# Mahdi-Si/VAE-TEB

Hardware: AMD Instinct MI355X
Metric: train samples/sec + ELBO, 4096-pt windows, batch 256, 1/2/4/8 MI355X (higher is better)
Workload: dtype bf16 MFMA (decoder heads + conv blocks + ResidualMLP linears, LSTM recurrences f16 fwd / bf16 bwd), fp32 accumulation; fp32 LayerNorm / BatchNorm / LSTM state / front-end / optimizer

## Files before the change

include/vaeteb.h:

```cpp
#ifndef VAETEB_H
#define VAETEB_H

#include <stdint.h>

#ifdef __cplusplus
extern "C" {
#endif

#define VT_OK 0
#define VT_ERR_ARG (-1)
#define VT_ERR_LAYOUT (-2)
#define VT_ERR_HIP (-3)

#define VT_FFT_MAX_LDS 8192

const char* vt_last_error(void);
int vt_stream_fork(void* from, void* to);
int vt_stream_mark(void* stream, int* slot);
int vt_stream_wait_mark(void* stream, int slot);
int vt_abi_version(void);
int vt_arrive_reset(void* stream);
int vt_capture_info(void* stream, char* buf, int len);
int vt_set_h16_format(int fp16);
int vt_get_h16_format(void);


int vt_fe_spectrum(const float* x, int64_t rows, int N, int n_pad, int pad_left, int pad_mode, const void* tw,
                   void* xhat, void* stream);
int vt_fe_spectrum_rolled(const float* x, int64_t B, int64_t x_row_stride, int N, int n_pad, int pad_left,
                          int pad_mode, const int* shifts, int K, const void* tw, void* xhat, void* stream);

int vt_fe_lowpass(const float* x, int64_t rows, int64_t x_row_stride, int N, int n_pad, int pad_left,
                  const float* h0, int radius, int step, int start, int S, float* out, int64_t out_row_stride,
                  void* stream);

int vt_fe_wavelet(const void* xhat, int64_t B, int C, int n_pad, const float* psi, int n_items, const int* items,
                  const void* tw, int N, int pad_left, void* analytic, int n_slots, const float* h0, int radius,
                  int step, int start, int S, float* s1, int s1_channels, void* stream);

int vt_fe_pairs(const void* analytic, int64_t B, int n_slots, int N, int n_pad, int pad_left, int n_pairs,
                const int* slot_i, const int* slot_j, const float* power, const void* tw, const float* phi0, int dec,
                int start, int S, int pad_mode, float* out, void* stream);
int vt_fe_pairs_split(const void* analytic_i, int n_slots_i, const void* analytic_j, int n_slots_j, int64_t B, int K,
                      int N, int n_pad, int pad_left, int n_pairs, const int* slot_i, const int* slot_j,
                      const float* power, const void* tw, const float* phi0, int dec, int start, int S,
                      int pad_mode, float* out, void* stream);

int vt_fe_set_pairs_persist(int grid);
int vt_fe_set_pairs_direct(int on);
int vt_fe_set_pairs_half(int on);
int vt_fe_set_analytic_polar(int on);

int vt_fe_set_pairs_stamps(void* buf);

int vt_fe_normalize(const float* in, int64_t B, int C, int in_C, int S, const int* kind, const float* mean, const float* stdv,
                    float log_eps, float* out, int out_C, int out_off, void* stream);
int vt_fe_normalize_window(const float* in, int64_t B, int C, int in_C, int in_S, int s0, int S_len,
                           const int* kind, const float* mean, const float* stdv, float log_eps, float* out,
                           int out_C, int out_off, void* stream);
int vt_copy_cols(const float* src, int64_t rows, int ld_src, int src_col0, int ncols, float* dst, int ld_dst,
                 int dst_col0, void* stream);
int vt_clamp_bwd(const float* g, const float* x, int64_t n, float lo, float hi, float* gx, void* stream);
int vt_zero_ranges(float* base, int n, const int64_t* starts, const int64_t* ends, void* stream);
int vt_normalize_raw(const float* x, int64_t rows, int64_t row_stride, int N, float mean, float stdv, float* out,
                     void* stream);

#define VT_STATS_CHUNK_ROWS 32
#define VT_STATS_CHUNK_COLS 1024
int vt_stats_chunking(int* rows, int* cols);
int vt_stats_workspace_bytes(int64_t B, int C, int S_len, int64_t* bytes);
int vt_stats_accum(const float* in, int64_t B, int C, int in_C, int in_S, int s0, int S_len, const int* kind,
                   double log_eps, int64_t* count, double* sum, double* sum_sq, void* work, int64_t work_bytes,
                   void* stream);
int vt_stats_accum_raw(const float* x, int64_t rows, int64_t row_stride, int N, int64_t* count, double* sum,
                       double* sum_sq, void* work, int64_t work_bytes, void* stream);

int vt_window_flat_stats(const float* base, const int64_t* row_off, int64_t rows, int N, double tolerance,
                         int min_length, int32_t* out, void* stream);
int vt_window_gather(const float* base, const int64_t* row_off, int64_t rows, int N, float* out, void* stream);

int vt_fft(const void* in, void* out, int64_t rows, int n, int inverse, const void* tw, int tw_stride,
           void* stream);
int vt_fft_large(const void* in, void* out, void* ws, int64_t rows, int n, int inverse, const void* tw,
                 void* stream);
int vt_cdgmm(const void* A, const void* B, int b_is_real, void* C, int64_t rows, int n, void* stream);
int vt_scat_filter_sub(const void* A, int B, int64_t a_rows, int n, const int* a_idx, const float* pool,
                       const int64_t* f_off, int P, int k, void* out, void* stream);
int vt_scat_mod_spec(const void* A, int B, int64_t a_rows, int n, const int* a_idx, const float* pool,
                     const int64_t* f_off, int P, int k, const void* tw, void* out, void* stream);
int vt_scat_lowpass(const void* U, int B, int P, int n, const float* phi, int k, int i0, int i1, const int* ch,
                    int out_C, const void* tw, float* out, void* stream);
int vt_modulus_cplx(const void* in, void* out, int64_t count, void* stream);
int vt_modulus(const void* in, float* out, int64_t count, void* stream);
int vt_modulus_bwd(const void* in, const float* mod, const float* grad, void* grad_in, int64_t count, void* stream);
int vt_subsample_fourier(const void* in, void* out, int64_t rows, int n, int k, void* stream);
int vt_pad_reflect(const float* in, float* out, int64_t rows, int N, int pad_left, int pad_right, void* stream);
int vt_scat_lowpass_bwd(const float* g, int B, int P, int n, const float* phi, int k, int i0, int i1, const int* ch,
                        int out_C, const void* tw, void* gU, void* stream);
int vt_scat_mod_spec_bwd(const void* A, int B, int64_t a_rows, int n, const int* a_idx, const float* pool,
                         const int64_t* f_off, int P, int k, const void* tw, const void* gUh, void* gX,
                         void* stream);
int vt_scat_fold_bwd(const void* gX, int B, int a_rows, int n, const int* csr_ptr, const int* csr_p,
                     const float* pool, const int64_t* f_off, int P, int k, void* gA, void* stream);
int vt_modulus_cplx_bwd(const void* z, const void* G, void* out, int64_t count, void* stream);
int vt_pad_reflect_bwd(const float* g, int g_stride, float scale, float* gx, int64_t rows, int N, int pad_left,
                       int pad_right, void* stream);
int vt_subsample_fourier_bwd(const void* g, void* gx, int64_t rows, int n, int k, void* stream);


int vt_elbo_workspace_floats(void);

int vt_elbo_latent_fwd(const float* mu_c, const float* lv_q, const float* mu_y, const float* lv_p, const float* eps,
                       int64_t rows, int D, float* z, float* mu_post, float* kl, float* ws, void* stream);
int vt_elbo_latent_bwd(const float* mu_c, const float* lv_q, const float* mu_y, const float* lv_p, const float* eps,
                       int64_t rows, int D, const float* g_z, const float* g_mu_post, const float* g_kl,
                       float* g_mu_c, float* g_lv_q, float* g_mu_y, float* g_lv_p, void* stream);
int vt_elbo_output_fwd(const float* mu, const float* lv, const float* y, int64_t n_nll, const float* lin,
                       const float* t_st, const float* t_ph, int64_t rows, int c_st, int c_ph, float* g_mu,
                       float* g_lv, float* g_lin, float* nll, float* mse, float* ws, void* stream);
int vt_scale_by_device_scalar(float* x, int64_t n, const float* s, void* stream);
int vt_te_kl_rows(const float* mu_c, const float* lv_q, const float* mu_y, const float* lv_p, int64_t B, int K,
                  int64_t row_elems, float* te, float* kl, void* stream);
int vt_eval_scale_rows(const float* x, int64_t B, int K, int64_t row_elems, const float* gains, float* out,
                       void* stream);
int vt_te_latent_rows(const float* mu_c, const float* lv_q, const float* mu_y, const float* lv_p, const float* eps,
                      int64_t B, int K, int64_t row_elems, float* z, float* mu_post, float* te, float* kl,
                      void* stream);
int vt_recon_metrics_rows(const float* y, const float* pr, int64_t B, int K, int64_t n, float* out, void* stream);

int vt_grad_norm_workspace_floats(void);
int vt_grad_norm_clip(const float* g, int64_t n, float pre_scale, float max_norm, float* out2, float* ws,
                      void* stream);
int vt_grad_norm_clip_scaled(const float* g, int64_t n, float pre_scale, float max_norm, float* out3, float* ws,
                             float* scaler, float growth_factor, float backoff_factor, int growth_interval,
                             void* stream);
int vt_adamw_step(float* p, const float* g, float* m, float* v, int64_t n, float lr, float beta1, float beta2,
                  float eps, float weight_decay, int step, const float* gscale, void* stream);
int vt_adamw_step_dev(float* p, const float* g, float* m, float* v, int64_t n, float lr, float beta1, float beta2,
                      float eps, float weight_decay, int* step, float* coef, const float* gscale, void* stream);
int vt_adamw_step_dev_shadow(float* p, const float* g, float* m, float* v, int64_t n, float lr, float beta1,
                             float beta2, float eps, float weight_decay, int* step, float* coef, const float* gscale,
                             int n_tiled, const int64_t* tiled_off, const int* tiled_N, const int* tiled_K,
                             const int64_t* tiled_w16, const int64_t* tiled_w16t, void* stream);
int vt_adamw_step_dev_skip(float* p, const float* g, float* m, float* v, int64_t n, float lr, float beta1,
                           float beta2, float eps, float weight_decay, int* step, float* coef, const float* gscale,
                           const float* skip, void* stream);
int vt_adamw_step_dev_shadow_skip(float* p, const float* g, float* m, float* v, int64_t n, float lr, float beta1,
                                  float beta2, float eps, float weight_decay, int* step, float* coef,
                                  const float* gscale, int n_tiled, const int64_t* tiled_off, const int* tiled_N,
                                  const int* tiled_K, const int64_t* tiled_w16, const int64_t* tiled_w16t,
                                  const float* skip, void* stream);
int vt_adamw_set_vector(int on);
int vt_cast_bf16(const float* src, void* dst, int64_t n, void* stream);
int vt_cast_bf16_to_f32(const void* src, float* dst, int64_t n, void* stream);

int vt_gemm_splits_hint(int64_t M, int N, int64_t K);
int vt_linear_fwd(const float* X, int64_t R, int K, const float* W, int N, const float* bias, float* Y, void* stream);
int vt_linear_bwd_data(const float* dY, int64_t R, int N, const float* W, int K, float* dX, int accumulate,
                       void* stream);
int vt_linear_bwd_weight(const float* dY, int64_t R, int N, const float* X, int K, float* dW, float* db,
                         int accumulate, float* ws, int64_t ws_floats, void* stream);
int vt_linear_ln_fwd(const float* X, int64_t R, int K, const float* W, int N, const float* bias, const float* gamma,
                     const float* beta, int act, float eps, float* Y, float* xhat, float* rstd, void* stream);
int vt_colsum(const float* X, int64_t R, int N, float* out, int accumulate, float* ws, int64_t ws_floats,
              void* stream);

#define VT_MLP_MAX_LAYERS 34
#define VT_MLP_MAX_WIDTH 144
int vt_resmlp_sizes(int n_layers, const int* dims, const int* layer_ln, const int* layer_act, int skip,
                    int64_t rows, int64_t* sizes);
int vt_resmlp_fwd(int n_layers, const int* dims, const int* layer_ln, const int* layer_act, int skip, float eps,
                  const float* const* params, const float* x, int64_t rows, float* out, float* xhat, float* rstd,
                  void* stream);
int vt_resmlp_bwd(int n_layers, const int* dims, const int* layer_ln, const int* layer_act, int skip, float eps,
                  const float* const* params, const float* dout, const float* xhat, const float* rstd, int64_t rows,
                  float* dx, float* const* grads, int accumulate, float* ws, int64_t ws_floats, void* stream);

int vt_resmlp_bf16_sizes(int n_layers, const int* dims, const int* layer_ln, const int* layer_act, int skip,
                         int64_t rows, int64_t* sizes);
int vt_resmlp_bf16_fwd(int n_layers, const int* dims, const int* layer_ln, const int* layer_act, int skip, float eps,
                       const float* const* params, const float* x, int64_t rows, float* out, float* xhat, float* rstd,
                       void* stream);
int vt_resmlp_bf16_bwd(int n_layers, const int* dims, const int* layer_ln, const int* layer_act, int skip, float eps,
                       const float* const* params, const float* dout, const float* xhat, const float* rstd,
                       int64_t rows, float* dx, float* const* grads, int accumulate, float* ws, int64_t ws_floats,
                       void* stream);
int vt_resmlp_bf16_plan(int n_layers, const int* dims, const int* layer_ln, const int* layer_act, int skip, float eps,
                        const float* const* params, int64_t rows, int64_t* handle, void* stream);
int vt_resmlp_bf16_prep_batch(int n, const int64_t* handles, void* stream);
int vt_resmlp_bf16_fwd_prepped(int n_layers, const int* dims, const int* layer_ln, const int* layer_act, int skip,
                               float eps, const float* const* params, const float* x, int64_t rows, float* out,
                               float* xhat, float* rstd, void* stream);
int vt_resmlp_bf16_split_sizes(int n_layers, const int* dims, const int* layer_ln, const int* layer_act, int skip,
                               int64_t rows, int64_t* sizes);
int vt_resmlp_bf16_bwd_data(int n_layers, const int* dims, const int* layer_ln, const int* layer_act, int skip,
                            float eps, const float* const* params, const float* dout, const float* xhat,
                            const float* rstd, int64_t rows, float* dx, float* const* grads, int accumulate,
                            void* dz16, float* ws, int64_t ws_floats, void* stream);
int vt_resmlp_bf16_bwd_weight(int n_layers, const int* dims, const int* layer_ln, const int* layer_act, int skip,
                              float eps, const float* const* params, const float* xhat, const void* dz16,
                              int64_t rows, float* const* grads, int accumulate, float* ws, int64_t ws_floats,
                              void* stream);
int vt_resmlp_bf16_set_stamps(void* buf);

int vt_mfma_supported(int K, int N);
int vt_mfma_workspace_floats(int64_t R, int K, int N, int64_t* floats);
int vt_mfma_weight_shadow(const float* W, int N, int K, void* W16, void* W16t, void* stream);
int vt_mfma_linear_fwd(const float* X, int64_t R, int K, const void* W16, int N, const float* bias, float* Y,
                       float* ws, int64_t ws_floats, void* stream);
int vt_mfma_linear_bwd_data(const float* dY, int64_t R, int N, const void* W16t, int K, float* dX, int accumulate,
                            float* ws, int64_t ws_floats, void* stream);
int vt_mfma_linear_bwd_weight(const float* dY, int64_t R, int N, const float* X, int K, float* dW, float* db,
                              int accumulate, float* ws, int64_t ws_floats, void* stream);

int vt_conv1d_out_len(int L_in, int K, int mode, int up);
int vt_conv1d_fwd(const float* X, int B, int L_in, int Cin, const float* W, int Cout, int K, int mode, int up,
                  float* Y, void* stream);
int vt_conv1d_bwd_data(const float* dY, int B, int L_in, int Cin, const float* W, int Cout, int K, int mode, int up,
                       float* dX, int accumulate, float* gpad, void* stream);
int vt_conv1d_bwd_weight(const float* dY, const float* X, int B, int L_in, int Cin, int Cout, int K, int mode, int up,
                         float* dW, int accumulate, float* ws, int64_t ws_floats, void* stream);
int vt_conv1d_bn_workspace_floats(int B, int L_in, int Cin, int Cout, int K, int mode, int up, int64_t* floats);
int vt_conv1d_bn_fwd(const float* X, int B, int L_in, int Cin, const float* W, int Cout, int K, int mode, int up,
                     const float* gamma, const float* beta, int act, float eps, float momentum, float* conv_out,
                     float* Y, float* mean, float* rstd, float* run_mean, float* run_var, float* ws,
                     int64_t ws_floats, void* stream);
int vt_conv1d_bf16_shadow(const float* W, int Cout, int Cin, int K, void* w16, void* w16t, void* stream);
int vt_conv1d_bf16_shadow_batch(int n, const int64_t* W, const int* Cout, const int* Cin, const int* K,
                                const int64_t* w16, const int64_t* w16t, void* stream);
int vt_conv_bf16_set_staging(int mode);
int vt_conv_bf16_set_kernels(int flags);
int vt_conv1d_bn_fwd_bf16(const float* X, int B, int L_in, int Cin, const void* w16, int Cout, int K, int mode,
                          int up, const float* gamma, const float* beta, int act, float eps, float momentum,
                          float* conv_out, float* Y, float* mean, float* rstd, float* run_mean, float* run_var,
                          float* ws, int64_t ws_floats, void* stream);
int vt_conv1d_bn_fwd_bf16_in(const float* X, const float* in_mean, const float* in_rstd, const float* in_gamma,
                             const float* in_beta, int in_act, int B, int L_in, int Cin, const void* w16, int Cout,
                             int K, int mode, int up, const float* gamma, const float* beta, int act, float eps,
                             float momentum, float* conv_out, float* Y, float* mean, float* rstd, float* run_mean,
                             float* run_var, float* ws, int64_t ws_floats, void* stream);
int vt_conv1d_fwd_bf16(const float* X, int B, int L_in, int Cin, const void* w16, int Cout, int K, int mode, int up,
                       float* Y, void* stream);
int vt_conv1d_bwd_gpad_bf16(const float* dY, int B, int L_in, int Cin, const void* w16t, int Cout, int K, int mode,
                            int up, float* gpad, void* stream);
int vt_conv1d_bwd_weight_bf16(const float* dY, const float* X, int B, int L_in, int Cin, int Cout, int K, int mode,
                              int up, float* dW, int accumulate, float* ws, int64_t ws_floats, void* stream);
int vt_conv1d_bwd_gpad_bf16_bn(const float* dY, const float* Xc, const float* bnp, int act, int64_t M, int B,
                               int L_in, int Cin, const void* w16t, int Cout, int K, int mode, int up, float* gpad,
                               void* dxbn16, void* stream);
int vt_conv1d_bwd_dx_bf16_bn(const float* dY, const float* Xc, const float* bnp, int act, int64_t M, int B, int L_in,
                             int Cin, const void* w16t, int Cout, int K, int mode, int up, float* dX, float* edge,
                             void* dxbn16, void* stream);
int vt_conv1d_bwd_weight_bf16_dy16(const void* dY16, const float* X, int B, int L_in, int Cin, int Cout, int K,
                                   int mode, int up, float* dW, int accumulate, float* ws, int64_t ws_floats,
                                   void* stream);
int vt_conv1d_bwd_weight_bf16_dy16s(const void* dY16, int dys, const float* X, int B, int L_in, int Cin, int Cout,
                                    int K, int mode, int up, float* dW, int accumulate, float* ws, int64_t ws_floats,
                                    void* stream);
int vt_conv1d_bwd_weight_bf16_in(const float* dY, const void* dY16, int dys, const float* X, const float* in_mean,
                                 const float* in_rstd, const float* in_gamma, const float* in_beta, int in_act, int B,
                                 int L_in, int Cin, int Cout, int K, int mode, int up, float* dW, int accumulate,
                                 float* ws, int64_t ws_floats, void* stream);
int vt_batchnorm_bwd_x16(const float* dY, const float* Xc, const float* bnp, int act, int64_t M, int C, void* d16,
                         void* stream);
int vt_conv1d_bwd_dx16(const void* d16, int B, int L_in, int Cin, const void* w16t, int Cout, int K, int mode, int up,
                       float* dX, float* edge, void* stream);
int vt_conv1d_direct_fwd(const float* X, int B, int L_in, int Cin, const float* W, int Cout, int K, int mode, int up,
                         float* Y, void* stream);
int vt_conv1d_direct_bwd_gpad(const float* dY, int B, int L_in, int Cin, const float* W, int Cout, int K, int mode,
                              int up, float* gpad, void* stream);
int vt_conv1d_fold(const float* gpad, int B, int L_in, int Cin, int Cout, int K, int mode, int up, float* dX,
                   int accumulate, void* stream);
int vt_conv1d_direct_bwd_weight(const float* dY, const float* X, int B, int L_in, int Cin, int Cout, int K, int mode,
                                int up, float* dW, int accumulate, float* ws, int64_t ws_floats, void* stream);

int vt_layernorm_fwd(const float* x, int64_t R, int C, const float* gamma, const float* beta, int act, float eps,
                     float* y, float* xhat, float* rstd, void* stream);
int vt_layernorm_bwd(const float* dy, const float* xhat, const float* rstd, int64_t R, int C, const float* gamma,
                     const float* beta, int act, float* dx, float* dgamma, float* dbeta, int accumulate_params,
                     float* ws, int64_t ws_floats, void* stream);
int vt_batchnorm_fwd(const float* x, int64_t M, int C, const float* gamma, const float* beta, int act, float eps,
                     float momentum, float* y, float* mean, float* rstd, float* run_mean, float* run_var, float* ws,
                     int64_t ws_floats, void* stream);
int vt_batchnorm_bwd(const float* dy, const float* x, int64_t M, int C, const float* mean, const float* rstd,
                     const float* gamma, const float* beta, int act, float* dx, float* dgamma, float* dbeta,
                     int accumulate_params, float* ws, int64_t ws_floats, void* stream);
int vt_batchnorm_fwd_dropout(const float* x, int64_t M, int C, const float* gamma, const float* beta, int act,
                             float eps, float momentum, float* y, float* mean, float* rstd, float* run_mean,
                             float* run_var, int L, float p, int64_t seed, const void* seed_offset, float* ws,
                             int64_t ws_floats, void* stream);
int vt_batchnorm_bwd_dropout(const float* dy, const float* x, int64_t M, int C, const float* mean, const float* rstd,
                             const float* gamma, const float* beta, int act, int L, float p, int64_t seed,
                             const void* seed_offset, float* dx, float* dgamma, float* dbeta, int accumulate_params,
                             float* ws, int64_t ws_floats, void* stream);
int vt_batchnorm_bwd_coef(const float* dy, const float* x, int64_t M, int C, const float* mean, const float* rstd,
                          const float* gamma, const float* beta, int act, float* dgamma, float* dbeta,
                          int accumulate_params, float* bnp, float* ws, int64_t ws_floats, void* stream);
int vt_batchnorm_eval(const float* x, int64_t M, int C, const float* run_mean, const float* run_var, float eps,
                      const float* gamma, const float* beta, int act, float* y, void* stream);
int vt_syncbn_sums(const float* x, const float* dy, int64_t M, int C, int which, const float* mean,
                   const float* rstd, const float* gamma, const float* beta, int act, double* sums, float* ws,
                   int64_t ws_floats, void* stream);
int vt_syncbn_stats(const double* sums, int C, int which, float eps, float momentum, float* mean, float* rstd,
                    float* run_mean, float* run_var, float* dgamma, float* dbeta, int accumulate, void* stream);
int vt_batchnorm_apply(const float* x, int64_t M, int C, const float* mean, const float* rstd, const float* gamma,
                       const float* beta, int act, float* y, void* stream);
int vt_syncbn_bwd_dx(const float* dy, const float* x, int64_t M, int C, const float* mean, const float* rstd,
                     const float* gamma, const float* beta, int act, const double* sums, float* dx, float* ws,
                     void* stream);
int vt_act_fwd(const float* x, int64_t n, int act, float* y, void* stream);
int vt_act_bwd(const float* dy, const float* x, int64_t n, int act, float* dx, void* stream);

int vt_lstm_layer_fwd(const float* gin, const float* w_hh, const float* b_hh, int B, int S, int hidden, float* out_h,
                      float* out_hprev, float* out_c, float* gates, void* stream);
int vt_lstm_layer_bwd(const float* dh_out, const float* gates, const float* cst, const float* w_hh, int B, int S,
                      int hidden, float* dgates, void* stream);
int vt_lstm_layer_fwd_x(const float* x, int In, const float* w_ih, const float* b_ih, const float* w_hh,
                        const float* b_hh, int B, int S, int hidden, float* out_h, float* out_hprev, float* out_c,
                        float* gates, void* stream);
int vt_lstm_layer_bwd_x(const float* dh_out, const float* gates, const float* cst, const float* w_hh,
                        const float* w_ih, int In, int B, int S, int hidden, float* dgates, float* dx, void* stream);
int vt_lstm16_layer_fwd(const float* x, int In, const float* w_ih, const float* b_ih, const float* w_hh,
                        const float* b_hh, int B, int S, int hidden, float* out_h, float* out_hprev, float* out_c,
                        float* gates, void* stream);
int vt_lstm16_layer_bwd(const float* dh_out, const float* gates, const float* cst, const float* w_hh,
                        const float* w_ih, int In, int B, int S, int hidden, float* dgates, float* dx, void* stream);
int vt_lstm16_pair_fwd(const float* x, int In, const float* w_ih0, const float* b_ih0, const float* w_hh0,
                       const float* b_hh0, const float* w_ih1, const float* b_ih1, const float* w_hh1,
                       const float* b_hh1, int B, int seq, int hidden, float* h0, float* c0, float* gates0, float* h1,
                       float* c1, float* gates1, void* stream);
int vt_lstm16_pair_bwd(const float* dh_out, const float* gates1, const float* c1, const float* w_hh1,
                       const float* w_ih1, const float* gates0, const float* c0, const float* w_hh0,
                       const float* w_ih0, int In0, int B, int seq, int hidden, void* dgates1, void* dgates0,
                       float* dx, void* stream, int dg_bf16);
int vt_lstm16_quad_fwd(const float* x, int In, const float* const* params, int B, int seq, int hidden,
                       float* const* outs, void* stream);
int vt_lstm16_quad_bwd(const float* dh_out, const float* const* w, const float* const* gc, int In0, int B, int seq,
                       int hidden, void* const* dg, float* dmid, float* dx, void* stream, int dg_bf16);
int vt_lstm16_chain_errors(int* count, int reset);
int vt_lstm_layer_bwd_weight(const float* dgates, const float* x, int In, const float* hprev, int B, int S,
                             int hidden, float* dw_ih, float* dw_hh, float* db_ih, float* db_hh, int accumulate,
                             float* ws, int64_t ws_floats, void* stream);
int vt_lstm16_layer_bwd_weight(const float* dgates, const float* x, int In, const float* h, int B, int S,
                               int hidden, float* dw_ih, float* dw_hh, float* db_ih, float* db_hh, int accumulate,
                               float* ws, int64_t ws_floats, void* stream);
int vt_lstm16_dg16_ok(int In);
int vt_lstm16_bwd_weight_multi(int nl, const void* const* dgates, const int* dg_bf16, const float* const* x,
                               const int* In, const float* const* h, int B, int seq, int hidden, float* const* grads,
                               const int* accumulate, float* ws, int64_t ws_floats, void* stream);

int vt_zconv_fwd(const float* X, int ldx, int B, int L, int Cin, const float* W, int Cout, int K, int pad_left,
                 float* Y, int ldy, int accumulate, void* stream);
int vt_zconv_bwd_data(const float* dY, int ldy, int B, int L, int Cin, const float* W, int Cout, int K, int pad_left,
                      float* dX, int ldx, int accumulate, void* stream);
int vt_zconv16_ws_floats(int Cin, int Cout, int K, int64_t* floats);
int vt_zconv16_fwd(const float* X, int ldx, int B, int L, int Cin, const float* W, int Cout, int K, int pad_left,
                   float* Y, int ldy, int accumulate, float* ws, int64_t ws_floats, void* stream);
int vt_zconv16_bwd_data(const float* dY, int ldy, int B, int L, int Cin, const float* W, int Cout, int K, int pad_left,
                        float* dX, int ldx, int accumulate, float* ws, int64_t ws_floats, void* stream);
int vt_zconv16_taps_elems(int Cin, int Cout, int K, int64_t* elems);
int vt_zconv16_taps(int n, const int64_t* W, const int* Cin, const int* Cout, const int* K, int flip,
                    const int64_t* T, void* stream);
int vt_zconv16_fwd_t(const float* X, int ldx, int B, int L, int Cin, const void* T, int Cout, int K, int pad_left,
                     float* Y, int ldy, int accumulate, void* stream);
int vt_zconv16_bwd_data_t(const float* dY, int ldy, int B, int L, int Cin, const void* T, int Cout, int K,
                          int pad_left, float* dX, int ldx, int accumulate, void* stream);
int vt_zconv16_bwd_weight(const float* dY, int ldy, const float* X, int ldx, int B, int L, int Cin, int Cout, int K,
                          int pad_left, float* dW, int accumulate, float* ws, int64_t ws_floats, void* stream);
int vt_zconv_bwd_weight_ws_floats(int B, int Cin, int Cout, int K, int64_t* floats);
int vt_zconv_bwd_weight(const float* dY, int ldy, const float* X, int ldx, int B, int L, int Cin, int Cout, int K,
                        int pad_left, float* dW, int accumulate, float* ws, int64_t ws_floats, void* stream);
int vt_maxpool3_fwd(const float* X, int B, int L, int C, float* Y, void* stream);
int vt_maxpool3_bwd(const float* dY, const float* X, int B, int L, int C, float* dX, int accumulate, void* stream);
int vt_add_act_fwd(const float* A, const float* Bm, int64_t n, int act, float* Y, void* stream);
int vt_add_act_dropout_fwd(const float* A, const float* Bm, int64_t n, int C, int act, int L, float p, int64_t seed,
                           const void* seed_offset, float* S_out, float* Y, void* stream);
int vt_act_dropout_bwd(const float* dY, const float* S_in, int64_t n, int C, int act, int L, float p, int64_t seed,
                       const void* seed_offset, float* dX, void* stream);
int vt_dropout_apply(const float* X, int64_t n, int C, int L, float p, int64_t seed, const void* seed_offset, float* Y,
                     void* stream);
int vt_dropout_seed_advance(void* offset, void* stream);
int vt_time_mean_fwd(const float* X, int B, int L, int C, float* Y, void* stream);
int vt_time_mean_bwd(const float* dY, int B, int L, int C, float* dX, int accumulate, void* stream);
int vt_attn_fwd(const float* qkv, int B, int S, int H, float scale, float p, int64_t seed, const void* seed_offset,
                float* out, float* lse, void* stream);
int vt_attn_bwd(const float* qkv, const float* out, const float* dout, const float* lse, int B, int S, int H,
                float scale, float p, int64_t seed, const void* seed_offset, float* dqkv, void* stream);
int vt_cross_entropy_fwd(const float* logits, const int64_t* labels, int B, int C, float* loss, float* probs,
                         void* stream);
int vt_cross_entropy_bwd(const float* probs, const int64_t* labels, int B, int C, const float* g, float* dlogits,
                         void* stream);

int vt_stepgraph_build(void* graph, int n_streams, void** handle);
int vt_stepgraph_launch(void* handle, void* const* streams);
int vt_stepgraph_info(void* handle, int* n_kernel, int* n_memcpy, int* n_memset, int* n_waits);
int vt_stepgraph_destroy(void* handle);
int vt_bucket_marker(int bucket, void* stream);
int vt_stepgraph_markers(void* handle, int* n_ops, int* n_markers, int* ends, int* buckets, int cap);
int vt_stepgraph_launch_range(void* handle, void* const* streams, int begin, int end, int flags);

#ifdef __cplusplus
}
#endif
#endif
```

vae-teb_amd/csrc/frontend.hip:

```cpp
#include <math.h>
#include <stdlib.h>

#include <mutex>
#include <vector>

#include "common.h"
#include "cfft.h"
#include "fft.h"

namespace vt {

static constexpr int FE_THREADS = 512;

__global__ __launch_bounds__(FE_THREADS) void k_fe_spectrum(const float* __restrict__ x, int N, int n_pad,
                                                            int pad_left, int pad_mode,
                                                            const float2* __restrict__ tw,
                                                            float2* __restrict__ xhat) {
    extern __shared__ __attribute__((aligned(16))) float2 sm[];
    float2* X = sm;
    float2* Y = sm + n_pad;
    const int64_t row = blockIdx.x;
    const float* xr = x + row * N;
    for (int n = threadIdx.x; n < n_pad; n += blockDim.x) {
        const int s = pad_src(n - pad_left, N, pad_mode);
        X[n] = make_float2(s < 0 ? 0.f : xr[s], 0.f);
    }
    __syncthreads();
    float2* R = fft_lds<false>(X, Y, n_pad, tw, 1);
    float2* o = xhat + row * n_pad;
    for (int n = threadIdx.x; n < n_pad; n += blockDim.x) o[n] = R[n];
}

__global__ __launch_bounds__(FE_THREADS) void k_fe_spectrum_rolled(const float* __restrict__ x, int64_t x_row_stride,
                                                                   int N, int n_pad, int pad_left, int pad_mode,
                                                                   const int* __restrict__ shifts, int K,
                                                                   const float2* __restrict__ tw,
                                                                   float2* __restrict__ xhat) {
    extern __shared__ __attribute__((aligned(16))) float2 sm[];
    float2* X = sm;
    float2* Y = sm + n_pad;
    const int64_t row = blockIdx.x;
    const float* xr = x + (row / K) * x_row_stride;
    int sh = shifts[row % K] % N;
    if (sh < 0) sh += N;
    for (int n = threadIdx.x; n < n_pad; n += blockDim.x) {
        const int s = pad_src(n - pad_left, N, pad_mode);
        int q = s - sh;
        if (q < 0) q += N;
        X[n] = make_float2(s < 0 ? 0.f : xr[q], 0.f);
    }
    __syncthreads();
    float2* R = fft_lds<false>(X, Y, n_pad, tw, 1);
    float2* o = xhat + row * n_pad;
    for (int n = threadIdx.x; n < n_pad; n += blockDim.x) o[n] = R[n];
}

__global__ __launch_bounds__(256) void k_fe_lowpass_lds(const float* __restrict__ x, int64_t x_row_stride, int N,
                                                        int n_pad, int pad_left, const float* __restrict__ h0,
                                                        int radius, int step, int start, int S,
                                                        float* __restrict__ out, int64_t out_row_stride) {
    extern __shared__ float xp[];
    const int64_t row = blockIdx.y;
    const float* xr = x + row * x_row_stride;
    const bool single = pad_left <= N - 1 && n_pad - pad_left - N <= N - 1;
    for (int n0 = threadIdx.x; n0 < n_pad; n0 += 256 * 8) {
        float v[8];
#pragma unroll
        for (int u = 0; u < 8; ++u) {
            const int n = n0 + 256 * u;
            const int i = n - pad_left;
            const int src = single ? (i < 0 ? -i : (i >= N ? 2 * N - 2 - i : i)) : reflect_idx(i, N);
            v[u] = n < n_pad ? xr[src] : 0.f;
        }
#pragma unroll
        for (int u = 0; u < 8; ++u)
            if (n0 + 256 * u < n_pad) xp[n0 + 256 * u] = v[u];
    }
    __syncthreads();
    const int m = blockIdx.x * 256 + threadIdx.x;
    if (m >= S) return;
    const int c = step * (m + start);
    float acc = 0.f;
    if (c - radius >= 0 && c + radius < n_pad) {
#pragma unroll 8
        for (int d = -radius; d <= radius; ++d) acc = fmaf(xp[c - d], h0[d < 0 ? -d : d], acc);
    } else {
        for (int d = -radius; d <= radius; ++d) {
            int n = (c - d) % n_pad;
            if (n < 0) n += n_pad;
            acc += xp[n] * h0[d < 0 ? -d : d];
        }
    }
    out[row * out_row_stride + m] = acc;
}

__global__ void k_fe_lowpass(const float* __restrict__ x, int64_t x_row_stride, int N, int n_pad, int pad_left,
                             const float* __restrict__ h0, int radius, int step, int start, int S,
                             float* __restrict__ out, int64_t out_row_stride) {
    const int64_t row = blockIdx.y;
    const int m = blockIdx.x * blockDim.x + threadIdx.x;
    if (m >= S) return;
    const float* xr = x + row * x_row_stride;
    const int c = step * (m + start);
    float acc = 0.f;
    for (int d = -radius; d <= radius; ++d) {
        int n = c - d;
        n %= n_pad;
        if (n < 0) n += n_pad;
        acc += xr[reflect_idx(n - pad_left, N)] * h0[d < 0 ? -d : d];
    }
    out[row * out_row_stride + m] = acc;
}

__global__ __launch_bounds__(FE_THREADS) void k_fe_wavelet(
    const float2* __restrict__ xhat, int C, int n_pad, const float* __restrict__ psi, int n_items,
    const int* __restrict__ items, const float2* __restrict__ tw, int N, int pad_left, float2* __restrict__ analytic,
    int n_slots, const float* __restrict__ h0, int radius, int step, int start, int S, float* __restrict__ s1,
    int s1_channels) {
    extern __shared__ __attribute__((aligned(16))) float2 sm[];
    float2* X = sm;
    float2* Y = sm + n_pad;
    const int item = blockIdx.x;
    const int64_t b = blockIdx.y;
    const int chan = items[item * 5 + 0], filt = items[item * 5 + 1], slot = items[item * 5 + 2];
    const int s1ch = items[item * 5 + 3], k1 = items[item * 5 + 4];
    const float2* xh = xhat + (b * C + chan) * n_pad;
    const float* ps = psi + (int64_t)filt * n_pad;
    for (int n = threadIdx.x; n < n_pad; n += blockDim.x) X[n] = cscale(xh[n], ps[n]);
    __syncthreads();
    float2* R = fft_lds<true>(X, Y, n_pad, tw, 1);
    const float inv_n = 1.0f / (float)n_pad;
    if (slot >= 0) {
        float2* a = analytic + (b * n_slots + slot) * (int64_t)N;
        for (int i = threadIdx.x; i < N; i += blockDim.x) a[i] = cscale(R[pad_left + i], inv_n);
    }
    if (s1ch >= 0) {
        float* U = reinterpret_cast<float*>(R == X ? Y : X);
        const int M = n_pad >> k1;
        for (int n = threadIdx.x; n < M; n += blockDim.x) {
            const float2 v = cscale(R[n << k1], inv_n);
            U[n] = sqrtf(v.x * v.x + v.y * v.y);
        }
        __syncthreads();
        for (int m = threadIdx.x; m < S; m += blockDim.x) {
            const int c = step * (m + start);
            const int lo = (c - radius + (1 << k1) - 1) >> k1;
            const int hi = (c + radius) >> k1;
            float acc = 0.f;
            for (int n = lo; n <= hi; ++n) {
                int d = c - (n << k1);
                d = d < 0 ? -d : d;
                int nn = n % M;
                if (nn < 0) nn += M;
                acc += U[nn] * h0[d];
            }
            s1[(b * s1_channels + s1ch) * S + m] = acc;
        }
    }
}

__device__ __forceinline__ float2 polar_rev(float2 a) {
    const float ax = fabsf(a.x), ay = fabsf(a.y);
    const float mx = fmaxf(ax, ay), mn = fminf(ax, ay);
    const float t = mx > 0.f ? mn * __builtin_amdgcn_rcpf(mx) : 0.f;
    const float s = t * t;
    float r = 0.000390918023f;
    r = fmaf(r, s, -0.00229176274f);
    r = fmaf(r, s, 0.00633099675f);
    r = fmaf(r, s, -0.0115143927f);
    r = fmaf(r, s, 0.016709527f);
    r = fmaf(r, s, -0.0225382969f);
    r = fmaf(r, s, 0.0318085626f);
    r = fmaf(r, s, -0.0530504771f);
    r = fmaf(r, s, 0.159154922f);
    r *= t;
    if (ay > ax) r = 0.25f - r;
    if (a.x < 0.f) r = 0.5f - r;
    r = copysignf(r, a.y);
    return make_float2(r, __builtin_amdgcn_sqrtf(a.x * a.x + a.y * a.y));
}
__device__ __forceinline__ float2 pair_polar(float2 pi, float2 pj, float p) {
    float v = fmaf(pi.x, p, -pj.x);
    v -= rintf(v);
    const float m = pi.y * pj.y;
    return make_float2(m * __builtin_amdgcn_cosf(v), m * __builtin_amdgcn_sinf(v));
}
template <bool POLAR>
__device__ __forceinline__ void fe_pairs_item(const float2* ai, const float2* aj, float* __restrict__ o, const float pw,
                                              int N, int n_pad, int pad_left, const float2* __restrict__ tw,
                                              const float* __restrict__ phi0, int dec, int start, int S,
                                              int pad_mode) {
    extern __shared__ __attribute__((aligned(16))) float2 sm[];
    float2* X = sm;
    float2* Y = sm + n_pad;
    for (int i = threadIdx.x; i < N; i += blockDim.x) {
        const float2 u = ai[i], v = aj[i];
        if constexpr (POLAR) {
            Y[i] = pair_polar(u, v, pw);
        } else {
            const float mag = sqrtf(u.x * u.x + u.y * u.y);
            const float ph = atan2f(u.y, u.x) * pw;
            float sn, cs;
            sincosf(ph, &sn, &cs);
            const float2 acc = make_float2(mag * cs, mag * sn);
            Y[i] = cmul(acc, cconj(v));
        }
        if (dec == 0) o[i] = Y[i].x;
    }
    if (dec == 0) return;
    __syncthreads();
    for (int n = threadIdx.x; n < n_pad; n += blockDim.x) {
        const int s = pad_src(n - pad_left, N, pad_mode);
        X[n] = s < 0 ? make_float2(0.f, 0.f) : Y[s];
    }
    __syncthreads();
    float2* R = fft_lds<false>(X, Y, n_pad, tw, 1);
    float2* Z = (R == X) ? Y : X;
    const int nb = n_pad / dec;
    for (int k = threadIdx.x; k < nb; k += blockDim.x) Z[k] = cscale(R[k], phi0[k]);
    __syncthreads();
    float2* Rs = fft_lds<true>(Z, R, nb, tw, dec);
    const float inv = 1.0f / (float)nb;
    for (int m = threadIdx.x; m < S; m += blockDim.x) o[m] = Rs[start + m].x * inv;
}

template <bool POLAR>
__global__ __launch_bounds__(FE_THREADS) void k_fe_pairs(
    const float2* __restrict__ analytic, int n_slots, int N, int n_pad, int pad_left, int n_pairs,
    const int* __restrict__ slot_i, const int* __restrict__ slot_j, const float* __restrict__ power,
    const float2* __restrict__ tw, const float* __restrict__ phi0, int dec, int start, int S, int pad_mode,
    float* __restrict__ out) {
    const int pair = blockIdx.x;
    const int64_t b = blockIdx.y;
    const float2* ai = analytic + (b * n_slots + slot_i[pair]) * (int64_t)N;
    const float2* aj = analytic + (b * n_slots + slot_j[pair]) * (int64_t)N;
    const float pw = power[pair];
    float* o = out + (b * n_pairs + pair) * (int64_t)S;
    fe_pairs_item<POLAR>(ai, aj, o, pw, N, n_pad, pad_left, tw, phi0, dec, start, S, pad_mode);
}

template <bool POLAR>
__global__ __launch_bounds__(FE_THREADS) void k_fe_pairs_split(
    const float2* __restrict__ analytic_i, int n_slots_i, const float2* __restrict__ analytic_j, int n_slots_j, int K,
    int N, int n_pad, int pad_left, int n_pairs, const int* __restrict__ slot_i, const int* __restrict__ slot_j,
    const float* __restrict__ power, const float2* __restrict__ tw, const float* __restrict__ phi0, int dec,
    int start, int S, int pad_mode, float* __restrict__ out) {
    const int pair = blockIdx.x;
    const int64_t r = blockIdx.y;
    const float2* ai = analytic_i + ((r / K) * n_slots_i + slot_i[pair]) * (int64_t)N;
    const float2* aj = analytic_j + (r * n_slots_j + slot_j[pair]) * (int64_t)N;
    const float pw = power[pair];
    float* o = out + (r * n_pairs + pair) * (int64_t)S;
    fe_pairs_item<POLAR>(ai, aj, o, pw, N, n_pad, pad_left, tw, phi0, dec, start, S, pad_mode);
}

static constexpr int PR_N = 8192, PR_NB = 512, PR_IMG = 16 * 16 * 33;
static constexpr int PR_T = 512;

__device__ __forceinline__ int pr_pos(int idx) {
    return (idx >> 5) * 33 + (idx & 31);
}

__device__ __forceinline__ float2 accel(float2 a, float p) {
    const float ax = fabsf(a.x), ay = fabsf(a.y);
    const float mx = fmaxf(ax, ay), mn = fminf(ax, ay);
    const float t = mx > 0.f ? mn * __builtin_amdgcn_rcpf(mx) : 0.f;
    const float s = t * t;
    float r = 0.000390918023f;
    r = fmaf(r, s, -0.00229176274f);
    r = fmaf(r, s, 0.00633099675f);
    r = fmaf(r, s, -0.0115143927f);
    r = fmaf(r, s, 0.016709527f);
    r = fmaf(r, s, -0.0225382969f);
    r = fmaf(r, s, 0.0318085626f);
    r = fmaf(r, s, -0.0530504771f);
    r = fmaf(r, s, 0.159154922f);
    r *= t;
    if (ay > ax) r = 0.25f - r;
    if (a.x < 0.f) r = 0.5f - r;
    r = copysignf(r, a.y);
    float v = r * p;
    v -= rintf(v);
    const float mag = __builtin_amdgcn_sqrtf(a.x * a.x + a.y * a.y);
    return make_float2(mag * __builtin_amdgcn_cosf(v), mag * __builtin_amdgcn_sinf(v));
}

template <bool POLAR>
__device__ __forceinline__ float2 pair_prod(float2 ai, float2 aj, float p) {
    if constexpr (POLAR) return pair_polar(ai, aj, p);
    else return F2(pmulc(C2(accel(ai, p)), C2(aj)));
}

__device__ __forceinline__ int xcd_item(int L, int total) {
    return (total & 7) == 0 ? (L & 7) * (total >> 3) + (L >> 3) : L;
}

#define PR_STAMP(i)                                                              \
    do {                                                                         \
        if constexpr (P) {                                                       \
            if (t == 0) stamps[((int64_t)b * n_pairs + pair) * 8 + (i)] = wall_clock64(); \
        }                                                                        \
    } while (0)
static constexpr int PR_ZP = PR_NB + PR_NB / 8;
template <bool G, bool D, bool P, bool POLAR>
__device__ __forceinline__ void fe_pairs8k_item(const float2* ai, const float2* aj, float* __restrict__ out,
                                                const float pw, int N_, int pad_left_,
                                                const float2* __restrict__ tab, const float* __restrict__ phi0,
                                                int start, int S, int pad_mode_, const int64_t b, int n_pairs,
                                                const int pair, unsigned long long* __restrict__ stamps) {
    static_assert(PR_T == 512, "one padded column per thread");
    const int N = G ? 4096 : N_, pad_left = G ? 2048 : pad_left_, pad_mode = G ? 0 : pad_mode_;
    extern __shared__ __attribute__((aligned(16))) float2 sm[];
    float2* img = sm;
    float2* Z = sm + PR_IMG;
    const int t = threadIdx.x;
    const int j3 = t & 255, ka = t >> 8, k2_3 = j3 >> 4, kb_3 = j3 & 15;
    const int k3 = k2_3 + 16 * kb_3 + 256 * ka;
    const float ph3 = phi0[k3];
    PR_STAMP(0);
    c2 v[16], w[15];
    auto load_w1 = [&]() {
#pragma unroll
        for (int k2 = 1; k2 < 16; ++k2) w[k2 - 1] = C2(tab[TW8K_T1 + 512 * (k2 - 1) + t]);
    };
    if constexpr (D) {
        load_w1();
        static_assert(G, "direct columns: training geometry");
        float2 xa[16], xb[16];
#pragma unroll
        for (int n2 = 0; n2 < 16; ++n2) {
            const int i = t + 512 * n2 - 2048;
            const int s = n2 < 4 ? -i : (n2 < 12 ? i : 2 * 4096 - 2 - i);
            xa[n2] = ai[s];
            xb[n2] = aj[s];
        }
#pragma unroll
        for (int n2 = 0; n2 < 16; ++n2) v[n2] = C2(pair_prod<POLAR>(xa[n2], xb[n2], pw));
    } else {
        for (int u0 = t; u0 < N; u0 += PR_T * 8) {
            float2 xa[8], xb[8];
#pragma unroll
            for (int k = 0; k < 8; ++k) {
                const int u = u0 + PR_T * k;
                xa[k] = (G || u < N) ? ai[u] : make_float2(0.f, 0.f);
                xb[k] = (G || u < N) ? aj[u] : make_float2(0.f, 0.f);
            }
#pragma unroll
            for (int k = 0; k < 8; ++k) {
                const int u = u0 + PR_T * k;
                if (G || u < N) img[u] = pair_prod<POLAR>(xa[k], xb[k], pw);
            }
        }
        PR_STAMP(1);
        load_w1();
        __syncthreads();
        const bool single = pad_mode == 0 && pad_left <= N - 1 && PR_N - pad_left - N <= N - 1;
#pragma unroll
        for (int n2 = 0; n2 < 16; ++n2) {
            const int i = t + 512 * n2 - pad_left;
            const int s = G ? (n2 < 4 ? -i : (n2 < 12 ? i : 2 * N - 2 - i))
                            : single ? (i < 0 ? -i : (i >= N ? 2 * N - 2 - i : i)) : pad_src(i, N, pad_mode);
            v[n2] = s < 0 ? c2{0.f, 0.f} : C2(img[s]);
        }
        __syncthreads();
    }
    {
        pdft16(v);
        img[pr_pos(t)] = F2(v[0]);
#pragma unroll
        for (int k2 = 1; k2 < 16; ++k2) img[pr_pos(t + 512 * k2)] = F2(pmul(v[k2], w[k2 - 1]));
    }
    PR_STAMP(2);
#pragma unroll
    for (int kb = 1; kb < 16; ++kb) w[kb - 1] = C2(tab[TW8K_T2 + 32 * (kb - 1) + (t & 31)]);
    __syncthreads();
    {
        const int k2 = t >> 5, n1a = t & 31;
        float2* base = img + k2 * 528 + n1a;
        c2 x[16];
#pragma unroll
        for (int n1b = 0; n1b < 16; ++n1b) x[n1b] = C2(base[33 * n1b]);
        pdft16(x);
        base[0] = F2(x[0]);
#pragma unroll
        for (int kb = 1; kb < 16; ++kb) base[33 * kb] = F2(pmul(x[kb], w[kb - 1]));
    }
    PR_STAMP(3);
    __syncthreads();
    {
        const float2* row = img + k2_3 * 528 + 33 * kb_3;
        c2 x = C2(row[0]);
        if (ka == 0) {
#pragma unroll
            for (int n1a = 1; n1a < 32; ++n1a) x += C2(row[n1a]);
        } else {
#pragma unroll
            for (int n1a = 1; n1a < 32; ++n1a) x = pmac(x, C2(row[n1a]), w32(n1a));
        }
        Z[z512_pos(k3)] = make_float2(x.x * ph3, -x.y * ph3);
    }
    PR_STAMP(4);
    c2 w5[7], wb5[7];
    if (t < 64) fft512_twiddles(tab, w5, wb5);
    __syncthreads();
    if (t < 64) {
        c2 r[8];
        wave_fft512(Z, w5, wb5, r);
        PR_STAMP(5);
        float* o = out + (b * n_pairs + pair) * (int64_t)S;
        const float inv = 1.0f / (float)PR_NB;
        const int k0 = (t >> 3) + 8 * (t & 7);
#pragma unroll
        for (int j = 0; j < 8; ++j) {
            const int m = k0 + 64 * j - start;
            if (m >= 0 && m < S) o[m] = r[j].x * inv;
        }
        PR_STAMP(6);
    }
}
#undef PR_STAMP

template <bool G, bool D = false, bool P = false, bool POLAR = true>
__global__ __launch_bounds__(PR_T) void k_fe_pairs8k(
    const float2* __restrict__ analytic, int n_slots, int N_, int pad_left_, int n_pairs, int B,
    const int* __restrict__ slot_i, const int* __restrict__ slot_j, const float* __restrict__ power,
    const float2* __restrict__ tab, const float* __restrict__ phi0, int start, int S, int pad_mode_,
    float* __restrict__ out, unsigned long long* __restrict__ stamps) {
    const int N = G ? 4096 : N_;
    const int item = xcd_item(blockIdx.x, n_pairs * B);
    const int pair = item % n_pairs;
    const int64_t b = item / n_pairs;
    const float2* ai = analytic + (b * n_slots + slot_i[pair]) * (int64_t)N;
    const float2* aj = analytic + (b * n_slots + slot_j[pair]) * (int64_t)N;
    const float pw = power[pair];
    fe_pairs8k_item<G, D, P, POLAR>(ai, aj, out, pw, N_, pad_left_, tab, phi0, start, S, pad_mode_, b, n_pairs, pair,
                                    stamps);
}

template <bool G, bool POLAR>
__global__ __launch_bounds__(PR_T) void k_fe_pairs8k_split(
    const float2* __restrict__ analytic_i, int n_slots_i, const float2* __restrict__ analytic_j, int n_slots_j, int K,
    int N_, int pad_left_, int n_pairs, int rows, const int* __restrict__ slot_i, const int* __restrict__ slot_j,
    const float* __restrict__ power, const float2* __restrict__ tab, const float* __restrict__ phi0, int start,
    int S, int pad_mode_, float* __restrict__ out) {
    const int N = G ? 4096 : N_;
    const int item = xcd_item(blockIdx.x, n_pairs * rows);
    const int pair = item % n_pairs;
    const int64_t r = item / n_pairs;
    const float2* ai = analytic_i + ((r / K) * n_slots_i + slot_i[pair]) * (int64_t)N;
    const float2* aj = analytic_j + (r * n_slots_j + slot_j[pair]) * (int64_t)N;
    const float pw = power[pair];
    fe_pairs8k_item<G, false, false, POLAR>(ai, aj, out, pw, N_, pad_left_, tab, phi0, start, S, pad_mode_, r,
                                            n_pairs, pair, nullptr);
}

static constexpr int PRP_T7 = PR_T - 64;
template <bool POLAR>
__device__ __forceinline__ void pr_product_w17(float2* img, const float2* __restrict__ ai,
                                               const float2* __restrict__ aj, float pw, int t7) {
#pragma unroll
    for (int bt = 0; bt < 2; ++bt) {
        float2 xa[5], xb[5];
#pragma unroll
        for (int k = 0; k < 5; ++k) {
            const int u = t7 + PRP_T7 * (5 * bt + k);
            if (bt == 0 || u < 4096) {
                xa[k] = ai[u];
                xb[k] = aj[u];
            }
        }
#pragma unroll
        for (int k = 0; k < 5; ++k) {
            const int u = t7 + PRP_T7 * (5 * bt + k);
            if (bt == 0 || u < 4096) img[u] = pair_prod<POLAR>(xa[k], xb[k], pw);
        }
    }
}

template <bool POLAR>
__global__ __launch_bounds__(PR_T) __attribute__((amdgpu_waves_per_eu(4, 4))) void k_fe_pairs8k_p(
    const float2* __restrict__ analytic, int n_slots, int n_pairs, int B, const int* __restrict__ slot_i,
    const int* __restrict__ slot_j, const float* __restrict__ power, const float2* __restrict__ tab,
    const float* __restrict__ phi0, int start, int S, float* __restrict__ out) {
    constexpr int N = 4096;
    extern __shared__ __attribute__((aligned(16))) float2 sm[];
    float2* img = sm;
    float2* Z = sm + PR_IMG;
    const int t = threadIdx.x, total = n_pairs * B;
    const int j3 = t & 255, ka = t >> 8, k2_3 = j3 >> 4, kb_3 = j3 & 15;
    const int k3 = k2_3 + 16 * kb_3 + 256 * ka;
    const float ph3 = phi0[k3];
    auto item_of = [&](int L, int& pair, int64_t& b) {
        const int item = xcd_item(L, total);
        pair = item % n_pairs;
        b = item / n_pairs;
    };
    int L = blockIdx.x;
    int pair;
    int64_t b;
    item_of(L, pair, b);
    if (t >= 64)
        pr_product_w17<POLAR>(img, analytic + (b * n_slots + slot_i[pair]) * (int64_t)N,
                       analytic + (b * n_slots + slot_j[pair]) * (int64_t)N, power[pair], t - 64);
    for (; L < total; L += gridDim.x) {
        __syncthreads();
        const float2* tb = tab;
        asm volatile("" : "+s"(tb));
        c2 v[16];
#pragma unroll
        for (int n2 = 0; n2 < 16; ++n2) {
            const int i = t + 512 * n2 - 2048;
            const int s = n2 < 4 ? -i : (n2 < 12 ? i : 2 * N - 2 - i);
            v[n2] = C2(img[s]);
        }
        __syncthreads();
        {
            c2 w[15];
#pragma unroll
            for (int k2 = 1; k2 < 16; ++k2) w[k2 - 1] = C2(tb[TW8K_T1 + 512 * (k2 - 1) + t]);
            pdft16(v);
            img[pr_pos(t)] = F2(v[0]);
#pragma unroll
            for (int k2 = 1; k2 < 16; ++k2) img[pr_pos(t + 512 * k2)] = F2(pmul(v[k2], w[k2 - 1]));
        }
        __syncthreads();
        {
            const int k2 = t >> 5, n1a = t & 31;
            float2* base = img + k2 * 528 + n1a;
            c2 w[15], x[16];
#pragma unroll
            for (int kb = 1; kb < 16; ++kb) w[kb - 1] = C2(tb[TW8K_T2 + 32 * (kb - 1) + n1a]);
#pragma unroll
            for (int n1b = 0; n1b < 16; ++n1b) x[n1b] = C2(base[33 * n1b]);
            pdft16(x);
            base[0] = F2(x[0]);
#pragma unroll
            for (int kb = 1; kb < 16; ++kb) base[33 * kb] = F2(pmul(x[kb], w[kb - 1]));
        }
        __syncthreads();
        {
            const float2* row = img + k2_3 * 528 + 33 * kb_3;
            c2 x = C2(row[0]);
            if (ka == 0) {
#pragma unroll
                for (int n1a = 1; n1a < 32; ++n1a) x += C2(row[n1a]);
            } else {
#pragma unroll
                for (int n1a = 1; n1a < 32; ++n1a) x = pmac(x, C2(row[n1a]), w32(n1a));
            }
            Z[z512_pos(k3)] = make_float2(x.x * ph3, -x.y * ph3);
        }
        __syncthreads();
        const int Ln = L + (int)gridDim.x;
        if (t < 64) {
            c2 r[8];
            wave_fft512(Z, tb, r);
            int st_ = start, S_ = S;
            asm volatile("" : "+s"(st_), "+s"(S_));
            float* o = out + (b * n_pairs + pair) * (int64_t)S_;
            const float inv = 1.0f / (float)PR_NB;
            const int k0 = (t >> 3) + 8 * (t & 7);
#pragma unroll
            for (int j = 0; j < 8; ++j) {
                const int m = k0 + 64 * j - st_;
                if (m >= 0 && m < S_) o[m] = r[j].x * inv;
            }
        } else if (Ln < total) {
            int np;
            int64_t nb;
            item_of(Ln, np, nb);
            pr_product_w17<POLAR>(img, analytic + (nb * n_slots + slot_i[np]) * (int64_t)N,
                           analytic + (nb * n_slots + slot_j[np]) * (int64_t)N, power[np], t - 64);
        }
        if (Ln < total) item_of(Ln, pair, b);
    }
}

static constexpr int PRH_IMG = 8 * 528;
static constexpr int PRH_BUF = PRH_IMG > 4096 ? PRH_IMG : 4096;
static constexpr int PRH_LDS = (PRH_BUF + PR_ZP) * (int)sizeof(float2);

__device__ __forceinline__ c2 w16c(int n) { return w32(2 * n); }

__device__ __forceinline__ float qx1(float v) {
    return __builtin_bit_cast(float, __builtin_amdgcn_update_dpp(0, __builtin_bit_cast(int, v), 0xB1, 0xF, 0xF, false));
}
__device__ __forceinline__ float qx2(float v) {
    return __builtin_bit_cast(float, __builtin_amdgcn_update_dpp(0, __builtin_bit_cast(int, v), 0x4E, 0xF, 0xF, false));
}

__device__ __forceinline__ int prh_src(int t, int n2) {
    const int i = t + 512 * n2 - 2048;
    return n2 < 4 ? -i : (n2 < 12 ? i : 2 * 4096 - 2 - i);
}

template <int H, int OCC, int P3>
__device__ __forceinline__ void prh_parity(float2* img, float2* Z, const c2 (&y)[8],
                                           const float2* __restrict__ tab, const float* __restrict__ phi0) {
    const int t = threadIdx.x, lane = t & 63;
    const int wv = __builtin_amdgcn_readfirstlane(t >> 6);
    float ph, ph1 = 0.f;
    if constexpr (P3 == 1) {
        const int k3 = (2 * (t >> 4) + H) + 16 * (t & 15);
        ph = t < 128 ? phi0[k3] : 0.f;
        ph1 = t < 128 ? phi0[k3 + 256] : 0.f;
    } else {
        ph = phi0[(2 * (t >> 6) + H) + 16 * ((t >> 2) & 15) + 256 * (t & 1)];
    }
#pragma unroll
    for (int m = 0; m < 8; ++m) img[528 * m + pr_pos(t)] = F2(y[m]);
    {
        const int p2 = wv & 1, n1a = lane & 31;
        float2* base = img + 528 * (2 * (wv >> 1) + (lane >> 5)) + n1a;
        c2 tw[8];
        auto load_tw = [&]() {
#pragma unroll
            for (int q = 0; q < 8; ++q) {
                const int kb = 2 * q + p2;
                if (kb > 0) tw[q] = C2(tab[TW8K_T2 + 32 * (kb - 1) + n1a]);
            }
        };
        if constexpr (OCC == 6) load_tw();
        __syncthreads();
        if constexpr (OCC != 6) load_tw();
        c2 x[8];
        if (p2 == 0) {
#pragma unroll
            for (int n = 0; n < 8; ++n) x[n] = C2(base[33 * n]) + C2(base[33 * (n + 8)]);
        } else {
#pragma unroll
            for (int n = 0; n < 8; ++n) {
                const c2 e = C2(base[33 * n]) - C2(base[33 * (n + 8)]);
                x[n] = n == 0 ? e : (n == 4 ? mul_mi(e) : pmul(e, w16c(n)));
            }
        }
        __syncthreads();
        pdft8(x);
        if (p2 == 0) {
            base[0] = F2(x[0]);
#pragma unroll
            for (int q = 1; q < 8; ++q) base[33 * 2 * q] = F2(pmul(x[q], tw[q]));
        } else {
#pragma unroll
            for (int q = 0; q < 8; ++q) base[33 * (2 * q + 1)] = F2(pmul(x[q], tw[q]));
        }
    }
    __syncthreads();
    if constexpr (P3 == 1) {
        if (t < 128) {
            const int m3 = t >> 4, kb3 = t & 15;
            const float2* row = img + 528 * m3 + 33 * kb3;
            c2 x0 = c2{0.f, 0.f}, x1 = c2{0.f, 0.f};
#pragma unroll
            for (int n = 0; n < 8; ++n) {
                const c2 a = C2(row[n]), b = C2(row[n + 8]), c = C2(row[n + 16]), e = C2(row[n + 24]);
                x0 += (a + c) + (b + e);
                const c2 f = add_mi(a - c, b - e);
                x1 = n == 0 ? f : pmac(x1, f, w32(n));
            }
            const int k3 = (2 * m3 + H) + 16 * kb3;
            Z[z512_pos(k3)] = make_float2(x0.x * ph, -x0.y * ph);
            Z[z512_pos(k3 + 256)] = make_float2(x1.x * ph1, -x1.y * ph1);
        }
    } else {
        const int q3 = t & 3, kb3 = (t >> 2) & 15;
        const float2* row = img + 528 * wv + 33 * kb3 + 8 * q3;
        c2 e0 = C2(row[0]), e1 = e0;
#pragma unroll
        for (int j = 1; j < 8; ++j) {
            const c2 v = C2(row[j]);
            e0 += v;
            e1 = pmac(e1, v, w32(j));
        }
        float rx = (q3 & 1) ? e1.y : e1.x, ry = (q3 & 1) ? -e1.x : e1.y;
        const float sg = (q3 & 2) ? -1.f : 1.f;
        rx *= sg;
        ry *= sg;
        float a0 = e0.x + qx1(e0.x), a1 = e0.y + qx1(e0.y), b0 = rx + qx1(rx), b1 = ry + qx1(ry);
        a0 += qx2(a0);
        a1 += qx2(a1);
        b0 += qx2(b0);
        b1 += qx2(b1);
        if (q3 < 2) {
            const int k3 = (2 * wv + H) + 16 * kb3 + 256 * q3;
            const float xr = q3 ? b0 : a0, xi = q3 ? b1 : a1;
            Z[z512_pos(k3)] = make_float2(xr * ph, -xi * ph);
        }
    }
}

template <bool POLAR, int OCC, int P3>
__device__ __forceinline__ void fe_pairs8k_h_item(const float2* ai, const float2* aj, float* __restrict__ o,
                                                  const float pw, const float2* __restrict__ tab,
                                                  const float* __restrict__ phi0, int start, int S) {
    extern __shared__ __attribute__((aligned(16))) float2 sm[];
    float2* img = sm;
    float2* Z = sm + PRH_BUF;
    const int t = threadIdx.x;
    constexpr int LB = OCC == 6 ? 8 : 4;
#pragma unroll
    for (int k0 = 0; k0 < 8; k0 += LB) {
        float2 xa[LB], xb[LB];
#pragma unroll
        for (int k = 0; k < LB; ++k) {
            xa[k] = ai[t + PR_T * (k0 + k)];
            xb[k] = aj[t + PR_T * (k0 + k)];
        }
#pragma unroll
        for (int k = 0; k < LB; ++k) img[t + PR_T * (k0 + k)] = pair_prod<POLAR>(xa[k], xb[k], pw);
    }
    __syncthreads();
    c2 s[8], d[8], w[8];
#pragma unroll
    for (int n = 0; n < 8; ++n) {
        const c2 va = C2(img[prh_src(t, n)]), vb = C2(img[prh_src(t, n + 8)]);
        s[n] = va + vb;
        d[n] = va - vb;
    }
#pragma unroll
    for (int n = 1; n < 8; ++n) d[n] = n == 4 ? mul_mi(d[n]) : pmul(d[n], w16c(n));
#pragma unroll
    for (int m = 1; m < 8; ++m) w[m] = C2(tab[TW8K_T1 + 512 * (2 * m - 1) + t]);
    pdft8(s);
#pragma unroll
    for (int m = 1; m < 8; ++m) s[m] = pmul(s[m], w[m]);
    __syncthreads();
    prh_parity<0, OCC, P3>(img, Z, s, tab, phi0);
#pragma unroll
    for (int m = 0; m < 8; ++m) w[m] = C2(tab[TW8K_T1 + 512 * (2 * m) + t]);
    pdft8(d);
#pragma unroll
    for (int m = 0; m < 8; ++m) d[m] = pmul(d[m], w[m]);
    __syncthreads();
    prh_parity<1, OCC, P3>(img, Z, d, tab, phi0);
    c2 w5[7], wb5[7];
    if (t < 64) fft512_twiddles(tab, w5, wb5);
    __syncthreads();
    if (t < 64) {
        c2 r[8];
        wave_fft512(Z, w5, wb5, r);
        const float inv = 1.0f / (float)PR_NB;
        const int k0 = (t >> 3) + 8 * (t & 7);
#pragma unroll
        for (int j = 0; j < 8; ++j) {
            const int m = k0 + 64 * j - start;
            if (m >= 0 && m < S) o[m] = r[j].x * inv;
        }
    }
}

template <bool POLAR, int OCC, int P3 = 1>
__global__ __launch_bounds__(PR_T) __attribute__((amdgpu_waves_per_eu(OCC, OCC))) void k_fe_pairs8k_h(
    const float2* __restrict__ analytic, int n_slots, int n_pairs, int B, const int* __restrict__ slot_i,
    const int* __restrict__ slot_j, const float* __restrict__ power, const float2* __restrict__ tab,
    const float* __restrict__ phi0, int start, int S, float* __restrict__ out) {
    constexpr int N = 4096;
    const int item = xcd_item(blockIdx.x, n_pairs * B);
    const int pair = item % n_pairs;
    const int64_t b = item / n_pairs;
    const float2* ai = analytic + (b * n_slots + slot_i[pair]) * (int64_t)N;
    const float2* aj = analytic + (b * n_slots + slot_j[pair]) * (int64_t)N;
    const float pw = power[pair];
    fe_pairs8k_h_item<POLAR, OCC, P3>(ai, aj, out + (b * n_pairs + pair) * (int64_t)S, pw, tab, phi0, start, S);
}

template <bool POLAR, int OCC, int P3 = 1>
__global__ __launch_bounds__(PR_T) __attribute__((amdgpu_waves_per_eu(OCC, OCC))) void k_fe_pairs8k_h_split(
    const float2* __restrict__ analytic_i, int n_slots_i, const float2* __restrict__ analytic_j, int n_slots_j, int K,
    int n_pairs, int rows, const int* __restrict__ slot_i, const int* __restrict__ slot_j,
    const float* __restrict__ power, const float2* __restrict__ tab, const float* __restrict__ phi0, int start,
    int S, float* __restrict__ out) {
    constexpr int N = 4096;
    const int item = xcd_item(blockIdx.x, n_pairs * rows);
    const int pair = item % n_pairs;
    const int64_t r = item / n_pairs;
    const float2* ai = analytic_i + ((r / K) * n_slots_i + slot_i[pair]) * (int64_t)N;
    const float2* aj = analytic_j + (r * n_slots_j + slot_j[pair]) * (int64_t)N;
    const float pw = power[pair];
    fe_pairs8k_h_item<POLAR, OCC, P3>(ai, aj, out + (r * n_pairs + pair) * (int64_t)S, pw, tab, phi0, start, S);
}

__device__ __forceinline__ int nat_pos(int k) { return k + (k >> 5); }

template <bool POLAR, bool LP = true>
__global__ __launch_bounds__(PR_T) void k_fe_wavelet8k(
    const float2* __restrict__ xhat, int C, const float* __restrict__ psi, const int* __restrict__ items, int n_items,
    int B, const float2* __restrict__ tab, int N, int pad_left, float2* __restrict__ analytic, int n_slots,
    const float* __restrict__ h0, int radius, int step, int start, int S, float* __restrict__ s1, int s1_channels,
    int nowrap) {
    static_assert(PR_T == 512, "one column per thread");
    extern __shared__ __attribute__((aligned(16))) float2 sm[];
    float2* img = sm;
    const int t = threadIdx.x;
    const int L = xcd_item(blockIdx.x, n_items * B);
    const int item = L % n_items;
    const int64_t b = L / n_items;
    const int chan = items[item * 5 + 0], filt = items[item * 5 + 1], slot = items[item * 5 + 2];
    const int s1ch = items[item * 5 + 3], k1 = items[item * 5 + 4];
    const float2* xh = xhat + (b * C + chan) * (int64_t)PR_N;
    const float* ps = psi + (int64_t)filt * PR_N;
    {
        c2 v[16], w[15];
#pragma unroll
        for (int n2 = 0; n2 < 16; ++n2) {
            const int n = t + 512 * n2;
            const float2 x = xh[n];
            const float p = ps[n];
            v[n2] = c2{x.x * p, -x.y * p};
        }
#pragma unroll
        for (int k2 = 1; k2 < 16; ++k2) w[k2 - 1] = C2(tab[TW8K_T1 + 512 * (k2 - 1) + t]);
        pdft16(v);
        img[pr_pos(t)] = F2(v[0]);
#pragma unroll
        for (int k2 = 1; k2 < 16; ++k2) img[pr_pos(t + 512 * k2)] = F2(pmul(v[k2], w[k2 - 1]));
    }
    c2 w2[15];
#pragma unroll
    for (int kb = 1; kb < 16; ++kb) w2[kb - 1] = C2(tab[TW8K_T2 + 32 * (kb - 1) + (t & 31)]);
    __syncthreads();
    {
        const int k2 = t >> 5, n1a = t & 31;
        float2* base = img + k2 * 528 + n1a;
        c2 x[16];
        const c2* w = w2;
#pragma unroll
        for (int n1b = 0; n1b < 16; ++n1b) x[n1b] = C2(base[33 * n1b]);
        pdft16(x);
        base[0] = F2(x[0]);
#pragma unroll
        for (int kb = 1; kb < 16; ++kb) base[33 * kb] = F2(pmul(x[kb], w[kb - 1]));
    }
    __syncthreads();
    const int k2 = (t & 255) >> 4, kb = t & 15;
    c2 r[32];
    if (t < 256) {
        const float2* row = img + k2 * 528 + 33 * kb;
#pragma unroll
        for (int n1a = 0; n1a < 32; ++n1a) r[n1a] = C2(row[n1a]);
        pdft32(r);
    }
    __syncthreads();
    const float inv_n = 1.0f / (float)PR_N;
    if (t < 256) {
#pragma unroll
        for (int ka = 0; ka < 32; ++ka) {
            const int k = k2 + 16 * kb + 256 * ka;
            img[nat_pos(k)] = make_float2(r[ka].x * inv_n, -r[ka].y * inv_n);
        }
    }
    __syncthreads();
    if (slot >= 0) {
        float2* a = analytic + (b * n_slots + slot) * (int64_t)N;
        for (int i = t; i < N; i += PR_T) {
            const float2 v = img[nat_pos(pad_left + i)];
            a[i] = POLAR ? polar_rev(v) : v;
        }
    }
    if (LP && s1ch >= 0) {
        const int M = PR_N >> k1;
        float* hl = reinterpret_cast<float*>(img + PR_IMG);
        for (int i = t; i <= radius; i += PR_T) hl[i] = h0[i];
        __syncthreads();
        for (int n = t; n < M; n += PR_T) {
            const float2 u = img[nat_pos(n << k1)];
            img[nat_pos(n << k1)].x = sqrtf(u.x * u.x + u.y * u.y);
        }
        __syncthreads();
        auto taps = [&](int c, int n0, int n1) {
            float acc = 0.f;
            for (int n = n0; n <= n1; ++n) {
                int d = c - (n << k1);
                d = d < 0 ? -d : d;
                int nn = n;
                if (!nowrap) {
                    nn %= M;
                    if (nn < 0) nn += M;
                }
                acc += img[nat_pos(nn << k1)].x * hl[d];
            }
            return acc;
        };
        if (nowrap && (step >> k1 << k1) == step) {
            const int jr = radius >> k1;
            for (int m = t; m < S; m += PR_T) {
                const int c0 = (step >> k1) * (m + start);
                float acc = 0.f;
#pragma unroll 8
                for (int j = -jr; j <= jr; ++j) {
                    const int nn = c0 + j;
                    acc = fmaf(img[nat_pos(nn << k1)].x, h0[(j < 0 ? -j : j) << k1], acc);
                }
                s1[(b * s1_channels + s1ch) * S + m] = acc;
            }
        } else {
            for (int m = t; m < S; m += PR_T) {
                const int c = step * (m + start);
                const int lo = (c - radius + (1 << k1) - 1) >> k1;
                const int hi = (c + radius) >> k1;
                s1[(b * s1_channels + s1ch) * S + m] = taps(c, lo, hi);
            }
        }
    } else if (s1ch >= 0) {
        const int M = PR_N >> k1;
        for (int m = t; m < S; m += PR_T) {
            const int c = step * (m + start);
            const int lo = (c - radius + (1 << k1) - 1) >> k1;
            const int hi = (c + radius) >> k1;
            float acc = 0.f;
            for (int n = lo; n <= hi; ++n) {
                int d = c - (n << k1);
                d = d < 0 ? -d : d;
                int nn = n;
                if (!nowrap) {
                    nn %= M;
                    if (nn < 0) nn += M;
                }
                const float2 u = img[nat_pos(nn << k1)];
                acc += sqrtf(u.x * u.x + u.y * u.y) * h0[d];
            }
            s1[(b * s1_channels + s1ch) * S + m] = acc;
        }
    }
}

__global__ void k_fe_normalize(const float* __restrict__ in, int C, int in_C, int in_S, int s0, int S,
                               const int* __restrict__ kind, const float* __restrict__ mean,
                               const float* __restrict__ stdv, float log_eps, float* __restrict__ out, int out_C,
                               int out_off) {
    const int64_t b = blockIdx.y;
    const int idx = blockIdx.x * blockDim.x + threadIdx.x;
    if (idx >= C * S) return;
    const int c = idx % C, s = idx / C;
    float v = in[(b * in_C + c) * in_S + s0 + s];
    const int k = kind[c];
    if (k == 1) v = logf(fmaxf(v, 0.f) + log_eps);
    else if (k == 2) v = asinhf(v);
    out[(b * S + s) * out_C + out_off + c] = (v - mean[c]) / (stdv[c] + 1e-8f);
}

__global__ void k_normalize_raw(const float* __restrict__ x, int64_t row_stride, int N, float mean, float stdv,
                                float* __restrict__ out) {
    const int64_t r = blockIdx.y;
    const int i = blockIdx.x * blockDim.x + threadIdx.x;
    if (i < N) out[r * N + i] = (x[r * row_stride + i] - mean) / (stdv + 1e-8f);
}

__global__ __launch_bounds__(FE_THREADS) void k_fft_rows(const float2* __restrict__ in, float2* __restrict__ out,
                                                         int n, const float2* __restrict__ tw, int tw_stride,
                                                         int inverse) {
    extern __shared__ __attribute__((aligned(16))) float2 sm[];
    float2* X = sm;
    float2* Y = sm + n;
    const int64_t r = blockIdx.x;
    for (int i = threadIdx.x; i < n; i += blockDim.x) X[i] = in[r * n + i];
    __syncthreads();
    float2* R = inverse ? fft_lds<true>(X, Y, n, tw, tw_stride) : fft_lds<false>(X, Y, n, tw, tw_stride);
    const float sc = inverse ? 1.0f / (float)n : 1.0f;
    for (int i = threadIdx.x; i < n; i += blockDim.x) out[r * n + i] = cscale(R[i], sc);
}

constexpr int F4_N1 = 256, F4_COLS = 16;

__global__ __launch_bounds__(FE_THREADS) void k_fft4_cols(const float2* __restrict__ in, float2* __restrict__ ws,
                                                          int n, int n2, const float2* __restrict__ tw, int inverse) {
    extern __shared__ __attribute__((aligned(16))) float2 sm[];
    constexpr int P = F4_N1 + 1;
    float2* X = sm;
    float2* Y = sm + F4_COLS * P;
    const int64_t r = blockIdx.y;
    const int c0 = blockIdx.x * F4_COLS;
    const float2* src = in + r * n + c0;
    for (int i = threadIdx.x; i < F4_N1 * F4_COLS; i += blockDim.x) {
        const int j1 = i / F4_COLS, c = i % F4_COLS;
        X[c * P + j1] = src[(int64_t)j1 * n2 + c];
    }
    __syncthreads();
    float2* R = inverse ? fft_lds_batch<true>(X, Y, F4_N1, F4_COLS, P, tw, n2)
                        : fft_lds_batch<false>(X, Y, F4_N1, F4_COLS, P, tw, n2);
    float2* dst = ws + r * n + c0;
    for (int i = threadIdx.x; i < F4_N1 * F4_COLS; i += blockDim.x) {
        const int k1 = i / F4_COLS, c = i % F4_COLS;
        const int e = (int)(((int64_t)(c0 + c) * k1) & (n - 1));
        const float2 w = inverse ? twiddle<true>(tw, e) : twiddle<false>(tw, e);
        dst[(int64_t)k1 * n2 + c] = cmul(R[c * P + k1], w);
    }
}

__global__ __launch_bounds__(FE_THREADS) void k_fft4_rows(const float2* __restrict__ ws, float2* __restrict__ out,
                                                          int n, int n2, int rb, const float2* __restrict__ tw,
                                                          int inverse) {
    extern __shared__ __attribute__((aligned(16))) float2 sm[];
    const int P = n2 + 1;
    float2* X = sm;
    float2* Y = sm + rb * P;
    const int64_t r = blockIdx.y;
    const int k10 = blockIdx.x * rb;
    const float2* src = ws + r * n + (int64_t)k10 * n2;
    for (int i = threadIdx.x; i < rb * n2; i += blockDim.x) {
        const int rr = i / n2, j2 = i - rr * n2;
        X[rr * P + j2] = src[i];
    }
    __syncthreads();
    float2* R = inverse ? fft_lds_batch<true>(X, Y, n2, rb, P, tw, F4_N1)
                        : fft_lds_batch<false>(X, Y, n2, rb, P, tw, F4_N1);
    const float sc = inverse ? 1.0f / (float)n : 1.0f;
    float2* dst = out + r * n + k10;
    for (int i = threadIdx.x; i < rb * n2; i += blockDim.x) {
        const int k2 = i / rb, rr = i - k2 * rb;
        dst[(int64_t)k2 * F4_N1 + rr] = cscale(R[rr * P + k2], sc);
    }
}

__global__ void k_cdgmm(const float2* __restrict__ A, const float* __restrict__ Bf, int b_real,
                        float2* __restrict__ C, int64_t total, int n) {
    const int64_t i = (int64_t)blockIdx.x * blockDim.x + threadIdx.x;
    if (i >= total) return;
    const int k = (int)(i % n);
    const float2 a = A[i];
    C[i] = b_real ? cscale(a, Bf[k]) : cmul(a, reinterpret_cast<const float2*>(Bf)[k]);
}

__global__ void k_modulus(const float2* __restrict__ in, float* __restrict__ out, int64_t total) {
    const int64_t i = (int64_t)blockIdx.x * blockDim.x + threadIdx.x;
    if (i < total) {
        const float2 v = in[i];
        out[i] = sqrtf(v.x * v.x + v.y * v.y);
    }
}

__global__ void k_modulus_bwd(const float2* __restrict__ in, const float* __restrict__ mod,
                              const float* __restrict__ g, float2* __restrict__ gin, int64_t total) {
    const int64_t i = (int64_t)blockIdx.x * blockDim.x + threadIdx.x;
    if (i < total) {
        const float m = mod[i];
        gin[i] = m == 0.f ? make_float2(0.f, 0.f) : cscale(in[i], g[i] / m);
    }
}

__global__ void k_subsample_fourier(const float2* __restrict__ in, float2* __restrict__ out, int64_t rows, int n,
                                    int k) {
    const int m = n / k;
    const int64_t i = (int64_t)blockIdx.x * blockDim.x + threadIdx.x;
    if (i >= rows * m) return;
    const int64_t r = i / m;
    const int j = (int)(i % m);
    float2 acc = make_float2(0.f, 0.f);
    for (int c = 0; c < k; ++c) acc = cadd(acc, in[r * n + c * m + j]);
    out[i] = cscale(acc, 1.0f / (float)k);
}

__global__ void k_pad_reflect(const float* __restrict__ in, float* __restrict__ out, int64_t rows, int N,
                              int pad_left, int n_out) {
    const int64_t i = (int64_t)blockIdx.x * blockDim.x + threadIdx.x;
    if (i >= rows * n_out) return;
    const int64_t r = i / n_out;
    const int j = (int)(i % n_out);
    out[i] = in[r * N + reflect_idx(j - pad_left, N)];
}

static inline bool pow2(int n) { return n > 0 && (n & (n - 1)) == 0; }

static const float2* tw8k_tables(hipStream_t st) {
    static std::mutex mu;
    static float2* tabs[64] = {};
    int dev = 0;
    if (hipGetDevice(&dev) != hipSuccess || dev < 0 || dev >= 64) return nullptr;
    std::lock_guard<std::mutex> lk(mu);
    if (tabs[dev] == nullptr) {
        hipStreamCaptureStatus cs = hipStreamCaptureStatusNone;
        if (hipStreamIsCapturing(st, &cs) != hipSuccess || cs != hipStreamCaptureStatusNone) return nullptr;
        std::vector<float2> h(TW8K_N);
        auto w = [](long m, long n) {
            const double a = -2.0 * M_PI * (double)(m % n) / (double)n;
            return make_float2((float)cos(a), (float)sin(a));
        };
        for (int k = 1; k < 16; ++k)
            for (int n = 0; n < 512; ++n) h[TW8K_T1 + 512 * (k - 1) + n] = w((long)n * k, 8192);
        for (int k = 1; k < 16; ++k)
            for (int n = 0; n < 32; ++n) h[TW8K_T2 + 32 * (k - 1) + n] = w((long)n * k, 512);
        for (int q = 1; q < 8; ++q)
            for (int l = 0; l < 64; ++l) h[TW8K_TA + 64 * (q - 1) + l] = w((long)l * q, 512);
        for (int r = 1; r < 8; ++r)
            for (int l = 0; l < 8; ++l) h[TW8K_TB + 8 * (r - 1) + l] = w((long)l * r, 64);
        float2* d = nullptr;
        if (hipMalloc(&d, sizeof(float2) * TW8K_N) != hipSuccess) return nullptr;
        if (hipMemcpy(d, h.data(), sizeof(float2) * TW8K_N, hipMemcpyHostToDevice) != hipSuccess) {
            (void)hipFree(d);
            return nullptr;
        }
        tabs[dev] = d;
    }
    return tabs[dev];
}
static inline size_t fft_lds_bytes(int n) { return (size_t)2 * n * sizeof(float2); }

}

using namespace vt;

extern "C" {

int vt_fe_spectrum(const float* x, int64_t rows, int N, int n_pad, int pad_left, int pad_mode, const void* tw,
                   void* xhat, void* stream) {
    VT_CHECK_ARG(pow2(n_pad) && n_pad <= VT_FFT_MAX_LDS && n_pad >= N, "vt_fe_spectrum: n_pad=%d", n_pad);
    VT_CHECK_ARG(rows > 0 && N > 1 && pad_mode >= 0 && pad_mode <= 2, "vt_fe_spectrum: rows/N/pad_mode");
    hipLaunchKernelGGL(k_fe_spectrum, dim3((unsigned)rows), dim3(FE_THREADS), fft_lds_bytes(n_pad), S(stream), x, N,
                       n_pad, pad_left, pad_mode, (const float2*)tw, (float2*)xhat);
    VT_LAUNCH_CHECK("vt_fe_spectrum");
    return VT_OK;
}

int vt_fe_spectrum_rolled(const float* x, int64_t B, int64_t x_row_stride, int N, int n_pad, int pad_left,
                          int pad_mode, const int* shifts, int K, const void* tw, void* xhat, void* stream) {
    VT_CHECK_ARG(pow2(n_pad) && n_pad <= VT_FFT_MAX_LDS && n_pad >= N, "vt_fe_spectrum_rolled: n_pad=%d", n_pad);
    VT_CHECK_ARG(B > 0 && K > 0 && N > 1 && pad_mode >= 0 && pad_mode <= 2 && pad_left >= 0 && x_row_stride >= N,
                 "vt_fe_spectrum_rolled: B/K/N/pad/stride");
    VT_CHECK_ARG(B * K < (1ll << 31), "vt_fe_spectrum_rolled: grid");
    VT_CHECK_ARG(x != nullptr && shifts != nullptr && tw != nullptr && xhat != nullptr,
                 "vt_fe_spectrum_rolled: null pointer");
    hipLaunchKernelGGL(k_fe_spectrum_rolled, dim3((unsigned)(B * K)), dim3(FE_THREADS), fft_lds_bytes(n_pad),
                       S(stream), x, x_row_stride, N, n_pad, pad_left, pad_mode, shifts, K, (const float2*)tw,
                       (float2*)xhat);
    VT_LAUNCH_CHECK("vt_fe_spectrum_rolled");
    return VT_OK;
}

int vt_fe_lowpass(const float* x, int64_t rows, int64_t x_row_stride, int N, int n_pad, int pad_left,
                  const float* h0, int radius, int step, int start, int S_out, float* out, int64_t out_row_stride,
                  void* stream) {
    VT_CHECK_ARG(rows > 0 && S_out > 0 && radius >= 0, "vt_fe_lowpass: shape");
    dim3 grid((S_out + 255) / 256, (unsigned)rows);
    if ((size_t)n_pad * sizeof(float) <= 64 * 1024)
        hipLaunchKernelGGL(k_fe_lowpass_lds, grid, dim3(256), (size_t)n_pad * sizeof(float), S(stream), x, x_row_stride,
                           N, n_pad, pad_left, h0, radius, step, start, S_out, out, out_row_stride);
    else
        hipLaunchKernelGGL(k_fe_lowpass, grid, dim3(256), 0, S(stream), x, x_row_stride, N, n_pad, pad_left, h0,
                           radius, step, start, S_out, out, out_row_stride);
    VT_LAUNCH_CHECK("vt_fe_lowpass");
    return VT_OK;
}

static int g_polar = -1;
static bool analytic_polar(int n_pad, int N, int pad_left) {
    if (g_polar < 0) {
        const char* e = getenv("VAETEB_ANALYTIC_POLAR");
        g_polar = e && e[0] == '0' ? 0 : 1;
    }
    return g_polar && n_pad == PR_N && pad_left + N <= PR_N;
}

int vt_fe_set_analytic_polar(int on) {
    (void)analytic_polar(PR_N, 0, 0);
    const int prev = g_polar;
    g_polar = on ? 1 : 0;
    return prev;
}

int vt_fe_wavelet(const void* xhat, int64_t B, int C, int n_pad, const float* psi, int n_items, const int* items,
                  const void* tw, int N, int pad_left, void* analytic, int n_slots, const float* h0, int radius,
                  int step, int start, int S_out, float* s1, int s1_channels, void* stream) {
    VT_CHECK_ARG(pow2(n_pad) && n_pad <= VT_FFT_MAX_LDS, "vt_fe_wavelet: n_pad=%d", n_pad);
    VT_CHECK_ARG(B > 0 && n_items > 0, "vt_fe_wavelet: empty");
    VT_CHECK_ARG(step * start - radius >= 0, "vt_fe_wavelet: lowpass window leaves the padded support");
    if (n_pad == PR_N && pad_left + N <= PR_N) {
        const int nowrap = step * (start + S_out - 1) + radius < n_pad ? 1 : 0;
        const float2* tab = tw8k_tables(S(stream));
        VT_CHECK_ARG(tab != nullptr, "vt_fe_wavelet: twiddle tables unavailable (first call under stream capture?)");
        VT_CHECK_ARG((int64_t)n_items * B < (1ll << 31), "vt_fe_wavelet: grid");
        static const bool lp_env = !(getenv("VAETEB_WAVELET_LP") && getenv("VAETEB_WAVELET_LP")[0] == '0');
        const bool lp = lp_env && radius < 2048;
        const bool pol = analytic_polar(n_pad, N, pad_left);
        auto kern = pol ? (lp ? k_fe_wavelet8k<true, true> : k_fe_wavelet8k<true, false>)
                        : (lp ? k_fe_wavelet8k<false, true> : k_fe_wavelet8k<false, false>);
        const size_t lds = PR_IMG * sizeof(float2) + (lp ? (size_t)((radius + 4) / 4 * 4) * 4 : 0);
        hipLaunchKernelGGL(kern, dim3((unsigned)(n_items * B)), dim3(PR_T), lds,
                           S(stream), (const float2*)xhat, C, psi, items, n_items, (int)B, tab, N, pad_left,
                           (float2*)analytic, n_slots, h0, radius, step, start, S_out, s1, s1_channels, nowrap);
    } else {
        hipLaunchKernelGGL(k_fe_wavelet, dim3(n_items, (unsigned)B), dim3(FE_THREADS), fft_lds_bytes(n_pad),
                           S(stream), (const float2*)xhat, C, n_pad, psi, n_items, items, (const float2*)tw, N,
                           pad_left, (float2*)analytic, n_slots, h0, radius, step, start, S_out, s1, s1_channels);
    }
    VT_LAUNCH_CHECK("vt_fe_wavelet");
    return VT_OK;
}

static unsigned long long* g_pairs_stamps = nullptr;
static int g_pairs_persist = -1;
static int pairs_persist_grid() {
    if (g_pairs_persist < 0) {
        const char* e = getenv("VAETEB_PAIRS_PERSIST");
        int v = e ? atoi(e) : 0;
        if (v < 0) {
            int dev = 0, cus = 256;
            if (hipGetDevice(&dev) == hipSuccess)
                (void)hipDeviceGetAttribute(&cus, hipDeviceAttributeMultiprocessorCount, dev);
            v = 2 * cus;
        }
        g_pairs_persist = v / 8 * 8;
    }
    return g_pairs_persist;
}
static int g_pairs_direct = -1;
static int pairs_direct() {
    if (g_pairs_direct < 0) {
        const char* e = getenv("VAETEB_PAIRS_DIRECT");
        g_pairs_direct = e != nullptr && e[0] == '1';
    }
    return g_pairs_direct;
}

int vt_fe_set_pairs_persist(int grid) {
    const int prev = pairs_persist_grid();
    if (grid < 0) {
        int dev = 0, cus = 256;
        if (hipGetDevice(&dev) == hipSuccess) (void)hipDeviceGetAttribute(&cus, hipDeviceAttributeMultiprocessorCount, dev);
        grid = 2 * cus;
    }
    g_pairs_persist = grid / 8 * 8;
    return prev;
}

static int g_pairs_half = -1;
static int pairs_half() {
    if (g_pairs_half < 0) {
        const char* e = getenv("VAETEB_PAIRS_HALF");
        g_pairs_half = e != nullptr ? atoi(e) : 1;
    }
    return g_pairs_half;
}

int vt_fe_set_pairs_half(int on) {
    const int prev = pairs_half();
    g_pairs_half = on < 0 ? 0 : on;
    return prev;
}

int vt_fe_set_pairs_direct(int on) {
    const int prev = pairs_direct();
    g_pairs_direct = on ? 1 : 0;
    return prev;
}

int vt_fe_set_pairs_stamps(void* buf) {
    g_pairs_stamps = (unsigned long long*)buf;
    return VT_OK;
}

int vt_fe_pairs(const void* analytic, int64_t B, int n_slots, int N, int n_pad, int pad_left, int n_pairs,
                const int* slot_i, const int* slot_j, const float* power, const void* tw, const float* phi0, int dec,
                int start, int S_out, int pad_mode, float* out, void* stream) {
    VT_CHECK_ARG(pow2(n_pad) && n_pad <= VT_FFT_MAX_LDS, "vt_fe_pairs: n_pad=%d", n_pad);
    VT_CHECK_ARG(dec == 0 ? S_out == N : (dec >= 1 && pow2(dec) && n_pad / dec >= start + S_out),
                 "vt_fe_pairs: dec/start (decimation must be a power of two)");
    VT_CHECK_ARG(B > 0 && n_pairs > 0 && pad_mode >= 0 && pad_mode <= 2, "vt_fe_pairs: empty/pad_mode");
    if (dec == PR_N / PR_NB && n_pad == PR_N && start + S_out <= PR_NB && N <= PR_IMG) {
        const bool geo = N == 4096 && pad_left == 2048 && pad_mode == 0;
        const bool direct = pairs_direct() != 0;
        const bool pol = analytic_polar(n_pad, N, pad_left);
        auto kern = pol ? (geo ? (direct ? k_fe_pairs8k<true, true, false, true> : k_fe_pairs8k<true, false, false, true>)
                               : k_fe_pairs8k<false, false, false, true>)
                        : (geo ? (direct ? k_fe_pairs8k<true, true, false, false> : k_fe_pairs8k<true, false, false, false>)
                               : k_fe_pairs8k<false, false, false, false>);
        if (g_pairs_stamps != nullptr && geo && !direct)
            kern = pol ? k_fe_pairs8k<true, false, true, true> : k_fe_pairs8k<true, false, true, false>;
        const float2* tab = tw8k_tables(S(stream));
        VT_CHECK_ARG(tab != nullptr, "vt_fe_pairs: twiddle tables unavailable (first call under stream capture?)");
        VT_CHECK_ARG((int64_t)n_pairs * B < (1ll << 31), "vt_fe_pairs: grid");
        const int64_t total = (int64_t)n_pairs * B;
        const int pgrid = pairs_persist_grid();
        if (geo && !direct && g_pairs_stamps == nullptr && pgrid > 0 && total >= 2 * pgrid) {
            hipLaunchKernelGGL(pol ? k_fe_pairs8k_p<true> : k_fe_pairs8k_p<false>, dim3((unsigned)pgrid), dim3(PR_T),
                               (PR_IMG + PR_ZP) * sizeof(float2),
                               S(stream), (const float2*)analytic, n_slots, n_pairs, (int)B, slot_i, slot_j, power, tab,
                               phi0, start, S_out, out);
            VT_LAUNCH_CHECK("vt_fe_pairs");
            return VT_OK;
        }
        if (geo && !direct && g_pairs_stamps == nullptr && pairs_half()) {
            const int hf = pairs_half();
            hipLaunchKernelGGL(pol ? (hf == 2   ? k_fe_pairs8k_h<true, 8>
                                      : hf == 3 ? k_fe_pairs8k_h<true, 6, 0>
                                                : k_fe_pairs8k_h<true, 6>)
                                   : (hf == 2   ? k_fe_pairs8k_h<false, 8>
                                      : hf == 3 ? k_fe_pairs8k_h<false, 6, 0>
                                                : k_fe_pairs8k_h<false, 6>),
                               dim3((unsigned)total), dim3(PR_T),
                               PRH_LDS, S(stream), (const float2*)analytic, n_slots, n_pairs, (int)B, slot_i, slot_j,
                               power, tab, phi0, start, S_out, out);
            VT_LAUNCH_CHECK("vt_fe_pairs");
            return VT_OK;
        }
        hipLaunchKernelGGL(kern, dim3((unsigned)(n_pairs * B)), dim3(PR_T), (PR_IMG + PR_ZP) * sizeof(float2),
                           S(stream), (const float2*)analytic, n_slots, N, pad_left, n_pairs, (int)B, slot_i, slot_j,
                           power, tab, phi0, start, S_out, pad_mode, out, g_pairs_stamps);
        if (g_pairs_stamps != nullptr && geo && !direct) g_pairs_stamps += (size_t)B * n_pairs * 8;
    } else {
        hipLaunchKernelGGL(analytic_polar(n_pad, N, pad_left) ? k_fe_pairs<true> : k_fe_pairs<false>,
                           dim3(n_pairs, (unsigned)B), dim3(FE_THREADS), fft_lds_bytes(n_pad), S(stream),
                           (const float2*)analytic, n_slots, N, n_pad, pad_left, n_pairs, slot_i, slot_j, power,
                           (const float2*)tw, phi0, dec, start, S_out, pad_mode, out);
    }
    VT_LAUNCH_CHECK("vt_fe_pairs");
    return VT_OK;
}

int vt_fe_pairs_split(const void* analytic_i, int n_slots_i, const void* analytic_j, int n_slots_j, int64_t B, int K,
                      int N, int n_pad, int pad_left, int n_pairs, const int* slot_i, const int* slot_j,
                      const float* power, const void* tw, const float* phi0, int dec, int start, int S_out,
                      int pad_mode, float* out, void* stream) {
    VT_CHECK_ARG(pow2(n_pad) && n_pad <= VT_FFT_MAX_LDS, "vt_fe_pairs_split: n_pad=%d", n_pad);
    VT_CHECK_ARG(dec == 0 ? S_out == N : (dec >= 1 && pow2(dec) && n_pad / dec >= start + S_out),
                 "vt_fe_pairs_split: dec/start (decimation must be a power of two)");
    VT_CHECK_ARG(B > 0 && K > 0 && n_pairs > 0 && n_slots_i > 0 && n_slots_j > 0 && N > 0 && pad_mode >= 0 &&
                     pad_mode <= 2,
                 "vt_fe_pairs_split: empty/pad_mode");
    VT_CHECK_ARG(analytic_i != nullptr && analytic_j != nullptr && slot_i != nullptr && slot_j != nullptr &&
                     power != nullptr && phi0 != nullptr && out != nullptr,
                 "vt_fe_pairs_split: null pointer");
    const int64_t rows = B * K;
    VT_CHECK_ARG(rows * n_pairs < (1ll << 31), "vt_fe_pairs_split: grid");
    const float2 *Ai = (const float2*)analytic_i, *Aj = (const float2*)analytic_j;
    if (dec == PR_N / PR_NB && n_pad == PR_N && start + S_out <= PR_NB && N <= PR_IMG) {
        const bool geo = N == 4096 && pad_left == 2048 && pad_mode == 0;
        const bool pol = analytic_polar(n_pad, N, pad_left);
        const float2* tab = tw8k_tables(S(stream));
        VT_CHECK_ARG(tab != nullptr, "vt_fe_pairs_split: twiddle tables unavailable (first call under stream capture?)");
        const int64_t total = rows * n_pairs;
        const int pgrid = pairs_persist_grid();
        const bool persist = pgrid > 0 && total >= 2 * pgrid;
        const int hf = pairs_half();
        if (geo && !persist && hf) {
            hipLaunchKernelGGL(pol ? (hf == 2   ? k_fe_pairs8k_h_split<true, 8>
                                      : hf == 3 ? k_fe_pairs8k_h_split<true, 6, 0>
                                                : k_fe_pairs8k_h_split<true, 6>)
                                   : (hf == 2   ? k_fe_pairs8k_h_split<false, 8>
                                      : hf == 3 ? k_fe_pairs8k_h_split<false, 6, 0>
                                                : k_fe_pairs8k_h_split<false, 6>),
                               dim3((unsigned)total), dim3(PR_T), PRH_LDS, S(stream), Ai, n_slots_i, Aj, n_slots_j, K,
                               n_pairs, (int)rows, slot_i, slot_j, power, tab, phi0, start, S_out, out);
        } else {
            hipLaunchKernelGGL(pol ? (geo ? k_fe_pairs8k_split<true, true> : k_fe_pairs8k_split<false, true>)
                                   : (geo ? k_fe_pairs8k_split<true, false> : k_fe_pairs8k_split<false, false>),
                               dim3((unsigned)total), dim3(PR_T), (PR_IMG + PR_ZP) * sizeof(float2), S(stream), Ai,
                               n_slots_i, Aj, n_slots_j, K, N, pad_left, n_pairs, (int)rows, slot_i, slot_j, power,
                               tab, phi0, start, S_out, pad_mode, out);
        }
    } else {
        VT_CHECK_ARG(tw != nullptr, "vt_fe_pairs_split: null twiddles");
        VT_CHECK_ARG(rows <= 65535, "vt_fe_pairs_split: rows=%lld > 65535 (grid y)", (long long)rows);
        hipLaunchKernelGGL(analytic_polar(n_pad, N, pad_left) ? k_fe_pairs_split<true> : k_fe_pairs_split<false>,
                           dim3(n_pairs, (unsigned)rows), dim3(FE_THREADS), fft_lds_bytes(n_pad), S(stream), Ai,
                           n_slots_i, Aj, n_slots_j, K, N, n_pad, pad_left, n_pairs, slot_i, slot_j, power,
                           (const float2*)tw, phi0, dec, start, S_out, pad_mode, out);
    }
    VT_LAUNCH_CHECK("vt_fe_pairs_split");
    return VT_OK;
}

int vt_fe_normalize_window(const float* in, int64_t B, int C, int in_C, int in_S, int s0, int S_len,
                           const int* kind, const float* mean, const float* stdv, float log_eps, float* out,
                           int out_C, int out_off, void* stream) {
    VT_CHECK_ARG(B > 0 && C > 0 && S_len > 0 && out_off + C <= out_C && in_C >= C && s0 >= 0 && s0 + S_len <= in_S,
                 "vt_fe_normalize_window: shape");
    dim3 grid((C * S_len + 255) / 256, (unsigned)B);
    hipLaunchKernelGGL(k_fe_normalize, grid, dim3(256), 0, S(stream), in, C, in_C, in_S, s0, S_len, kind, mean, stdv,
                       log_eps, out, out_C, out_off);
    VT_LAUNCH_CHECK("vt_fe_normalize_window");
    return VT_OK;
}

int vt_fe_normalize(const float* in, int64_t B, int C, int in_C, int S_len, const int* kind, const float* mean,
                    const float* stdv, float log_eps, float* out, int out_C, int out_off, void* stream) {
    return vt_fe_normalize_window(in, B, C, in_C, S_len, 0, S_len, kind, mean, stdv, log_eps, out, out_C, out_off,
                                  stream);
}

int vt_normalize_raw(const float* x, int64_t rows, int64_t row_stride, int N, float mean, float stdv, float* out,
                     void* stream) {
    VT_CHECK_ARG(rows > 0 && N > 0, "vt_normalize_raw: shape");
    dim3 grid((N + 255) / 256, (unsigned)rows);
    hipLaunchKernelGGL(k_normalize_raw, grid, dim3(256), 0, S(stream), x, row_stride, N, mean, stdv, out);
    VT_LAUNCH_CHECK("vt_normalize_raw");
    return VT_OK;
}

int vt_fft(const void* in, void* out, int64_t rows, int n, int inverse, const void* tw, int tw_stride,
           void* stream) {
    VT_CHECK_ARG(pow2(n) && n <= VT_FFT_MAX_LDS && rows > 0, "vt_fft: n=%d rows=%lld", n, (long long)rows);
    hipLaunchKernelGGL(k_fft_rows, dim3((unsigned)rows), dim3(FE_THREADS), fft_lds_bytes(n), S(stream),
                       (const float2*)in, (float2*)out, n, (const float2*)tw, tw_stride, inverse);
    VT_LAUNCH_CHECK("vt_fft");
    return VT_OK;
}

int vt_fft_large(const void* in, void* out, void* ws, int64_t rows, int n, int inverse, const void* tw,
                 void* stream) {
    VT_CHECK_ARG(pow2(n) && n > VT_FFT_MAX_LDS && n <= (1 << 21) && rows > 0 && rows <= 65535,
                 "vt_fft_large: n=%d rows=%lld (pow2, %d < n <= 2^21)", n, (long long)rows, VT_FFT_MAX_LDS);
    VT_CHECK_ARG(ws != in && ws != out, "vt_fft_large: workspace aliases in/out");
    const int n2 = n / F4_N1;
    int rb = 8192 / n2;
    if (rb > 16) rb = 16;
    hipStream_t st = S(stream);
    hipLaunchKernelGGL(k_fft4_cols, dim3(n2 / F4_COLS, (unsigned)rows), dim3(FE_THREADS),
                       (size_t)2 * F4_COLS * (F4_N1 + 1) * sizeof(float2), st, (const float2*)in, (float2*)ws, n, n2,
                       (const float2*)tw, inverse);
    hipLaunchKernelGGL(k_fft4_rows, dim3(F4_N1 / rb, (unsigned)rows), dim3(FE_THREADS),
                       (size_t)2 * rb * (n2 + 1) * sizeof(float2), st, (const float2*)ws, (float2*)out, n, n2, rb,
                       (const float2*)tw, inverse);
    VT_LAUNCH_CHECK("vt_fft_large");
    return VT_OK;
}

int vt_cdgmm(const void* A, const void* Bf, int b_is_real, void* Cout, int64_t rows, int n, void* stream) {
    VT_CHECK_ARG(rows > 0 && n > 0, "vt_cdgmm: shape");
    const int64_t total = rows * n;
    hipLaunchKernelGGL(k_cdgmm, dim3((unsigned)((total + 255) / 256)), dim3(256), 0, S(stream), (const float2*)A,
                       (const float*)Bf, b_is_real, (float2*)Cout, total, n);
    VT_LAUNCH_CHECK("vt_cdgmm");
    return VT_OK;
}

int vt_modulus(const void* in, float* out, int64_t count, void* stream) {
    VT_CHECK_ARG(count > 0, "vt_modulus: empty");
    hipLaunchKernelGGL(k_modulus, dim3((unsigned)((count + 255) / 256)), dim3(256), 0, S(stream), (const float2*)in,
                       out, count);
    VT_LAUNCH_CHECK("vt_modulus");
    return VT_OK;
}

int vt_modulus_bwd(const void* in, const float* mod, const float* grad, void* grad_in, int64_t count, void* stream) {
    VT_CHECK_ARG(count > 0, "vt_modulus_bwd: empty");
    hipLaunchKernelGGL(k_modulus_bwd, dim3((unsigned)((count + 255) / 256)), dim3(256), 0, S(stream),
                       (const float2*)in, mod, grad, (float2*)grad_in, count);
    VT_LAUNCH_CHECK("vt_modulus_bwd");
    return VT_OK;
}

int vt_subsample_fourier(const void* in, void* out, int64_t rows, int n, int k, void* stream) {
    VT_CHECK_ARG(rows > 0 && k >= 1 && n % k == 0, "vt_subsample_fourier: n=%d k=%d", n, k);
    const int64_t total = rows * (n / k);
    hipLaunchKernelGGL(k_subsample_fourier, dim3((unsigned)((total + 255) / 256)), dim3(256), 0, S(stream),
                       (const float2*)in, (float2*)out, rows, n, k);
    VT_LAUNCH_CHECK("vt_subsample_fourier");
    return VT_OK;
}

int vt_pad_reflect(const float* in, float* out, int64_t rows, int N, int pad_left, int pad_right, void* stream) {
    VT_CHECK_ARG(rows > 0 && N > 1 && pad_left >= 0 && pad_right >= 0, "vt_pad_reflect: shape");
    const int n_out = N + pad_left + pad_right;
    const int64_t total = rows * n_out;
    hipLaunchKernelGGL(k_pad_reflect, dim3((unsigned)((total + 255) / 256)), dim3(256), 0, S(stream), in, out, rows, N,
                       pad_left, n_out);
    VT_LAUNCH_CHECK("vt_pad_reflect");
    return VT_OK;
}

}
```

vae-teb_amd/vaeteb/frontend.py:

```python
import math

import numpy as np
import torch

from . import _lib
from .filter_bank import build_bank, lowpass_taps, padding, twiddles

FIELDS = ("fhr_st", "fhr_ph", "fhr_up_ph")


def _i32(a, dev):
    return torch.as_tensor(np.ascontiguousarray(a, dtype=np.int32), device=dev)


def _f32(a, dev):
    return torch.as_tensor(np.ascontiguousarray(a, dtype=np.float32), device=dev)


class FrontEndPlan:

    def __init__(self, J=11, Q=4, T=16, N=4096, device="cuda", tail_tol=1e-9):
        self.J, self.Q, self.T, self.N = J, Q, T, N
        self.device = torch.device(device)
        pd = padding(N, J, Q, T)
        self.pad = pd
        self.n_pad, self.pad_left, self.pad_right = pd.n_pad, pd.pad_left, pd.pad_right
        if self.n_pad > 8192:
            raise NotImplementedError(f"fused front-end holds one FFT in LDS (n_pad <= 8192), got {self.n_pad}")
        bank = build_bank(pd.J_pad, J, Q, T)
        self.bank = bank
        self.log2T = int(math.floor(math.log2(T)))
        self.step = 2 ** self.log2T
        self.start = pd.ind_start[self.log2T]
        self.S = pd.ind_end[self.log2T] - pd.ind_start[self.log2T]
        self.n_filters = len(bank.xi1)
        self.k1 = np.maximum(np.minimum(bank.j1, self.log2T), 0)

        xi = bank.xi1.astype(np.float32)
        ii, jj, pw = [], [], []
        for i in range(len(xi)):
            for j in range(len(xi)):
                if xi[j] >= xi[i]:
                    ii.append(i); jj.append(j)
                    pw.append(np.float32(xi[j]) / np.float32(xi[i]) if xi[i] > 1e-8 else np.float32(1.0))
        self.i_idx, self.j_idx = np.array(ii), np.array(jj)
        self.powers = np.array(pw, dtype=np.float32)
        self.autoc_idx = np.array([k for k in range(len(ii)) if ii[k] == jj[k]])
        self.center_freqs = xi
        self.phase_mask, self.cross_mask = self.fhr_masks()

        self.dec = max(1, min(N, N // self.S)) if N > self.S else 1
        self.nb = self.n_pad // self.dec
        self.pair_start = self.pad_left // self.dec
        self.pair_len = min(N // self.dec, self.nb - self.pair_start)
        h0, radius = lowpass_taps(bank.phi_levels[0], tail_tol)
        self.radius = radius

        dev = self.device
        self.t_psi = _f32(bank.psi1, dev)
        self.t_h0 = _f32(h0, dev)
        self.t_phi_crop = _f32(bank.phi_levels[0][: self.nb], dev)
        self.t_tw = _f32(twiddles(self.n_pad), dev)

    def fhr_masks(self):
        xi, pw, ii, jj = self.center_freqs, self.powers, self.i_idx, self.j_idx
        fmin = np.float32(0.006 if self.J >= 11 else 0.003)
        band = xi >= fmin
        auto = np.zeros(len(ii), bool)
        auto[self.autoc_idx] = True
        phase = band[ii] & band[jj] & auto
        for r in (2, 3):
            phase |= band[ii] & band[jj] & (np.abs(pw - np.float32(r)) < np.float32(0.1)) & (pw <= 8)
        up = xi < np.float32(0.02)
        fh = (xi >= np.float32(0.04)) & (xi <= np.float32(0.5))
        cross = up[ii] & fh[jj] & (pw >= 1) & (pw <= 32)
        return phase, cross

    def tables(self, phase_pairs, cross_pairs, scattering=True):
        need = set()
        for k in phase_pairs:
            need.add((0, int(self.i_idx[k]))); need.add((0, int(self.j_idx[k])))
        for k in cross_pairs:
            need.add((0, int(self.i_idx[k]))); need.add((1, int(self.j_idx[k])))
        slots = {cf: s for s, cf in enumerate(sorted(need))}
        items = []
        for f in range(self.n_filters):
            s1 = 1 + f if scattering else -1
            slot = slots.get((0, f), -1)
            if s1 >= 0 or slot >= 0:
                items.append((0, f, slot, s1, int(self.k1[f])))
        for f in range(self.n_filters):
            if (1, f) in slots:
                items.append((1, f, slots[(1, f)], -1, 0))
        pi = [slots[(0, int(self.i_idx[k]))] for k in phase_pairs] + \
             [slots[(0, int(self.i_idx[k]))] for k in cross_pairs]
        pj = [slots[(0, int(self.j_idx[k]))] for k in phase_pairs] + \
             [slots[(1, int(self.j_idx[k]))] for k in cross_pairs]
        pw = [self.powers[k] for k in phase_pairs] + [self.powers[k] for k in cross_pairs]
        dev = self.device
        return dict(n_slots=len(slots), items=_i32(np.array(items).reshape(-1, 5), dev), n_items=len(items),
                    slot_i=_i32(pi, dev), slot_j=_i32(pj, dev), power=_f32(pw, dev), n_pairs=len(pi))


PAD_MODES = {"reflect": 0, "constant": 1, "circular": 2}


def launch_spectrum(p, x, rows, pad_mode, xhat):
    _lib.call("vt_fe_spectrum", _lib.ptr(x), rows, p.N, p.n_pad, p.pad_left, pad_mode, _lib.ptr(p.t_tw),
              _lib.ptr(xhat), _lib.stream())


def launch_lowpass(p, x, rows, x_row_stride, out, out_row_stride):
    _lib.call("vt_fe_lowpass", _lib.ptr(x), rows, x_row_stride, p.N, p.n_pad, p.pad_left, _lib.ptr(p.t_h0), p.radius,
              p.step, p.start, p.S, out.data_ptr(), out_row_stride, _lib.stream())


def launch_wavelet(p, xhat, B, C, tab, analytic, s1, s1_channels):
    _lib.call("vt_fe_wavelet", _lib.ptr(xhat), B, C, p.n_pad, _lib.ptr(p.t_psi), tab["n_items"], _lib.ptr(tab["items"]),
              _lib.ptr(p.t_tw), p.N, p.pad_left, _lib.ptr(analytic) if analytic is not None else None,
              max(tab["n_slots"], 1), _lib.ptr(p.t_h0), p.radius, p.step, p.start, p.S,
              _lib.ptr(s1) if s1 is not None else None, s1_channels, _lib.stream())


def launch_pairs(p, analytic, B, tab, out, lowpass=True, pad_mode=0):
    if lowpass:
        _lib.call("vt_fe_pairs", _lib.ptr(analytic), B, tab["n_slots"], p.N, p.n_pad, p.pad_left, tab["n_pairs"],
                  _lib.ptr(tab["slot_i"]), _lib.ptr(tab["slot_j"]), _lib.ptr(tab["power"]), _lib.ptr(p.t_tw),
                  _lib.ptr(p.t_phi_crop), p.dec, p.pair_start, p.pair_len, pad_mode, _lib.ptr(out), _lib.stream())
    else:
        _lib.call("vt_fe_pairs", _lib.ptr(analytic), B, tab["n_slots"], p.N, p.n_pad, p.pad_left, tab["n_pairs"],
                  _lib.ptr(tab["slot_i"]), _lib.ptr(tab["slot_j"]), _lib.ptr(tab["power"]), _lib.ptr(p.t_tw),
                  _lib.ptr(p.t_phi_crop), 0, 0, p.N, pad_mode, _lib.ptr(out), _lib.stream())


class FrontEnd:

    def __init__(self, plan: FrontEndPlan, stats=None, trim=0):
        self.plan = p = plan
        if trim < 0 or 2 * trim >= p.S:
            raise ValueError(f"trim {trim} out of range for {p.S} steps")
        self.trim = trim
        self.S_out = p.S - 2 * trim
        self.N_out = p.N - 2 * trim * p.step
        self.phase_pairs = np.nonzero(p.phase_mask)[0]
        self.cross_pairs = np.nonzero(p.cross_mask)[0]
        self.tab = p.tables(self.phase_pairs, self.cross_pairs, scattering=True)
        self.C_st = 1 + p.n_filters
        self.C_ph, self.C_x = len(self.phase_pairs), len(self.cross_pairs)
        self.stats = None
        self.stats_accumulator = None
        if stats is not None:
            self.set_stats(stats)
        self._bufs = {}

    def set_stats(self, stats):
        dev = self.plan.device
        s = {}
        for f, n, kind in (("fhr_st", self.C_st, None), ("fhr_ph", self.C_ph, 2), ("fhr_up_ph", self.C_x, 2)):
            m = np.asarray(stats[f + "_mean"], np.float32).reshape(-1)
            v = np.asarray(stats[f + "_variance"], np.float32).reshape(-1)
            assert m.shape[0] == n, (f, m.shape, n)
            k = np.full(n, 2, np.int32) if kind == 2 else np.array([0] + [1] * (n - 1), np.int32)
            s[f] = (_i32(k, dev), _f32(m, dev), _f32(np.sqrt(v), dev))
        s["fhr"] = (float(np.asarray(stats["fhr_mean"])), float(np.sqrt(np.asarray(stats["fhr_variance"]))))
        self.stats = s

    def fit_stats(self, batches, side=None):
        from .stats import StatsAccumulator
        acc = StatsAccumulator.for_frontend(self)
        for x in batches:
            acc.update_windows(self, x, side)
        stats = acc.finalize()
        self.set_stats(stats)
        self.stats_accumulator = acc
        return stats

    def _buf(self, name, shape, dtype=torch.float32):
        b = self._bufs.get(name)
        if b is None or tuple(b.shape) != tuple(shape):
            b = torch.empty(shape, dtype=dtype, device=self.plan.device)
            self._bufs[name] = b
        return b

    def raw(self, x, side=None):
        p, t = self.plan, self.tab
        if x.dim() != 3 or x.shape[1] != 2 or x.shape[2] != p.N:
            raise ValueError(f"expected (B, 2, {p.N}) windows, got {tuple(x.shape)}")
        x = x.contiguous()
        B = x.shape[0]
        xhat = self._buf("xhat", (B, 2, p.n_pad, 2))
        launch_spectrum(p, x, B * 2, 0, xhat)
        s_raw = self._buf("s_raw", (B, self.C_st, p.S))
        launch_lowpass(p, x, B, 2 * p.N, s_raw, self.C_st * p.S)
        an = self._buf("analytic", (B, t["n_slots"], p.N, 2))
        launch_wavelet(p, xhat, B, 2, t, an, s_raw, self.C_st)
        if side is None or not self.C_ph or not self.C_x:
            pr = self._buf("pairs", (B, t["n_pairs"], p.pair_len))
            launch_pairs(p, an, B, t, pr, lowpass=True, pad_mode=0)
            return {"fhr_st": s_raw, "pairs": pr}
        main = torch.cuda.current_stream()
        side.wait_stream(main)
        pr = self._buf("pairs_ph", (B, self.C_ph, p.pair_len))
        launch_pairs(p, an, B, _sub_table(t, 0, self.C_ph), pr, lowpass=True, pad_mode=0)
        with torch.cuda.stream(side):
            px = self._buf("pairs_x", (B, self.C_x, p.pair_len))
            launch_pairs(p, an, B, _sub_table(t, self.C_ph, self.C_x), px, lowpass=True, pad_mode=0)
        return {"fhr_st": s_raw, "pairs": pr, "cross": px}

    def __call__(self, x, out=None, side=None):
        if self.stats is None:
            raise RuntimeError("FrontEnd needs normalisation statistics (set_stats)")
        p = self.plan
        r = self.raw(x, side)
        B, S, S0, Sl = x.shape[0], p.S, self.trim, self.S_out
        st = _lib.stream()
        out = {} if out is None else out
        get = lambda k, shape: out[k] if k in out else torch.empty(shape, device=p.device)
        y_st = get("fhr_st", (B, Sl, self.C_st))
        y_ph = get("fhr_ph", (B, Sl, self.C_ph))
        x_ph = get("fhr_up_ph", (B, Sl, self.C_x))
        y_raw = get("fhr", (B, self.N_out))
        k, m, s = self.stats["fhr_st"]
        _lib.call("vt_fe_normalize_window", _lib.ptr(r["fhr_st"]), B, self.C_st, self.C_st, S, S0, Sl, _lib.ptr(k),
                  _lib.ptr(m), _lib.ptr(s), 1e-6, _lib.ptr(y_st), self.C_st, 0, st)
        pairs = r["pairs"]
        if self.C_ph:
            k, m, s = self.stats["fhr_ph"]
            _lib.call("vt_fe_normalize_window", pairs.data_ptr(), B, self.C_ph, pairs.shape[1], S, S0, Sl,
                      _lib.ptr(k), _lib.ptr(m), _lib.ptr(s), 1e-6, _lib.ptr(y_ph), self.C_ph, 0, st)
        if self.C_x:
            k, m, s = self.stats["fhr_up_ph"]
            if "cross" in r:
                with torch.cuda.stream(side):
                    _lib.call("vt_fe_normalize_window", r["cross"].data_ptr(), B, self.C_x, self.C_x, S, S0, Sl,
                              _lib.ptr(k), _lib.ptr(m), _lib.ptr(s), 1e-6, _lib.ptr(x_ph), self.C_x, 0,
                              _lib.stream())
                x_ph.record_stream(side)
            else:
                _lib.call("vt_fe_normalize_window", pairs[:, self.C_ph:].data_ptr(), B, self.C_x, pairs.shape[1], S,
                          S0, Sl, _lib.ptr(k), _lib.ptr(m), _lib.ptr(s), 1e-6, _lib.ptr(x_ph), self.C_x, 0, st)
        fm, fs = self.stats["fhr"]
        _lib.call("vt_normalize_raw", _lib.ptr(x) + 4 * S0 * p.step, B, 2 * p.N, self.N_out, fm, fs, _lib.ptr(y_raw),
                  st)
        return {"fhr_st": y_st, "fhr_ph": y_ph, "fhr_up_ph": x_ph, "fhr": y_raw}


def _sub_table(t, first, count):
    s = dict(t)
    s["slot_i"], s["slot_j"], s["power"] = (t[k][first:first + count] for k in ("slot_i", "slot_j", "power"))
    s["n_pairs"] = count
    return s


def load_stats(J=11, Q=4, T=16, N=4096):
    import os
    path = os.path.join(os.path.dirname(__file__), "data", f"stats_j{J}q{Q}t{T}_n{N}.npz")
    return dict(np.load(path, allow_pickle=False))


class KymatioPhaseScattering1D(torch.nn.Module):

    def __init__(self, J, Q, T, shape, device=None, oversampling=0, max_order=2, border_mode="reflect",
                 tukey_alpha=None):
        super().__init__()
        if isinstance(Q, tuple):
            self.Q_scattering, self.Q = Q, Q[0]
        else:
            self.Q_scattering = self.Q = Q
        self.J, self.T, self.oversampling, self.max_order = J, T, oversampling, max_order
        self.border_mode, self.tukey_alpha = border_mode, tukey_alpha
        self.device = device if device is not None else torch.device("cuda")
        self.eps = 1e-14
        self.N = int(shape) if isinstance(shape, (int, float)) else int(shape[0])
        from .scattering import Scattering1D
        self.scattering = Scattering1D(J=J, shape=self.N, Q=self.Q, max_order=max_order, average=True,
                                       oversampling=oversampling, vectorize=True, out_type="array", T=T)
        self.plan = FrontEndPlan(J, self.Q, T, self.N, device=self.device)
        p = self.plan
        self.J_pad, self.pad_left, self.pad_right, self.N_padded = p.pad.J_pad, p.pad_left, p.pad_right, p.n_pad
        self.ind_start, self.ind_end = p.pad.ind_start, p.pad.ind_end
        self.center_freqs = torch.from_numpy(p.center_freqs).to(self.device)
        self.i_idx = torch.from_numpy(p.i_idx).to(self.device)
        self.j_idx = torch.from_numpy(p.j_idx).to(self.device)
        self.powers = torch.from_numpy(p.powers).to(self.device)
        self.autoc_idx = torch.from_numpy(p.autoc_idx).to(self.device)

    def get_optimal_coefficients_for_fhr(self, j_config=11, q_config=4, t_config=16):
        phase, cross = self.plan.fhr_masks()
        pm = torch.from_numpy(phase).to(self.device)
        cm = torch.from_numpy(cross).to(self.device)
        return {"phase_selection": {"optimal_mask": pm}, "cross_selection": {"cross_mask": cm},
                "recommendations": {"use_phase_mask": pm, "use_cross_mask": cm,
                                    "total_selected_features": j_config * q_config + 1 + int(pm.sum()) + int(cm.sum())}}

    def _tukey(self, x):
        a, n = self.tukey_alpha, x.shape[-1]
        if a is None or not (0 < a <= 1):
            return x
        if a >= 1.0:
            w = torch.hann_window(n, periodic=False, device=x.device)
        else:
            tl = int(a * (n - 1) / 2.0)
            if tl == 0:
                return x
            taper = torch.hann_window(2 * tl, periodic=False, device=x.device)
            w = torch.ones(n, device=x.device)
            w[:tl] = taper[:tl]
            w[n - tl:] = taper[tl:]
        return x * w

    def forward(self, x, compute_phase=True, compute_cross_phase=False, cross_phase_same_pairs_only=False,
                cross_phase_low_pass=True, scattering_channel=0, phase_channels=None):
        x = x.to(self.device).float()
        if self.tukey_alpha is not None:
            x = self._tukey(x)
        if x.dim() == 3:
            B, C, N = x.shape
            if scattering_channel >= C:
                raise ValueError(f"scattering_channel {scattering_channel} >= {C}")
            s_in = x[:, scattering_channel, :].contiguous()
            if compute_cross_phase:
                if phase_channels is None:
                    if C < 2:
                        raise ValueError("Cross-channel correlation requires at least 2 channels")
                    phase_channels = [0, 1]
                if len(phase_channels) != 2 or any(ch >= C for ch in phase_channels):
                    raise ValueError("Invalid phase_channels for cross-channel correlation")
                ph = x[:, phase_channels, :].contiguous()
            elif phase_channels is not None:
                if len(phase_channels) != 1:
                    raise ValueError("Single-channel phase correlation requires exactly 1 channel")
                if phase_channels[0] >= C:
                    raise ValueError(f"phase_channel {phase_channels[0]} >= {C}")
                ph = x[:, phase_channels[0], :].contiguous()
            else:
                ph = s_in
        elif x.dim() == 2:
            if scattering_channel != 0:
                raise ValueError("scattering_channel must be 0 for single-channel input")
            if compute_cross_phase:
                raise ValueError("Cross-channel correlation requires multi-channel input")
            s_in, ph = x.contiguous(), (x.contiguous() if compute_phase else None)
        else:
            raise ValueError(f"Input must be 2D or 3D, got shape {x.shape}")
        S, _ = self.scattering(s_in)
        res = {"scattering": S}
        if S.shape[-1] == 0:
            raise ValueError(f"Scattering output has zero temporal dimension: {S.shape}")
        if (compute_phase or compute_cross_phase) and ph is not None:
            if ph.dim() == 2:
                ph = ph.unsqueeze(1)
            if compute_cross_phase and ph.shape[1] != 2:
                raise ValueError("Cross-channel correlation requires exactly 2 channels")
            p = self.plan
            B, C = ph.shape[0], ph.shape[1]
            if compute_cross_phase:
                sel = self.autoc_idx.cpu().numpy() if cross_phase_same_pairs_only else np.arange(len(p.i_idx))
                tab = p.tables([], sel, scattering=False)
            else:
                tab = p.tables(np.arange(len(p.i_idx)), [], scattering=False)
            pm = PAD_MODES.get(self.border_mode)
            if pm is None:
                raise ValueError(f"Unsupported border_mode: {self.border_mode}")
            xhat = torch.empty((B, C, p.n_pad, 2), device=x.device)
            launch_spectrum(p, ph, B * C, pm, xhat)
            an = torch.empty((B, tab["n_slots"], p.N, 2), device=x.device)
            launch_wavelet(p, xhat, B, C, tab, an, None, 0)
            low = (not compute_cross_phase) or cross_phase_low_pass
            out = torch.empty((B, tab["n_pairs"], p.pair_len if low else p.N), device=x.device)
            launch_pairs(p, an, B, tab, out, lowpass=low, pad_mode=pm)
            res["cross_phase_corr" if compute_cross_phase else "phase_corr"] = out
            res["autoc_idx"] = self.autoc_idx
        return res
```

Baseline: 33660.

## Fuse front-end normalization epilogues into spectrum, lowpass, wavelet and pairs kernels

Adds an epilogue descriptor so the lowpass, wavelet and pairs kernels can apply the log/asinh plus mean/std normalization and trimmed-window transpose directly when storing results. It also folds raw-signal normalization into the spectrum kernel. This removes the separate normalize kernels and the intermediate pair and scattering buffers round-tripping through HBM. By default raw and pairs are fused while the scattering path is not. The cost is strided (transposed) stores from the FFT kernels and extra registers and a sync in the pairs kernels.

```diff
diff --git a/include/vaeteb.h b/include/vaeteb.h
--- a/include/vaeteb.h
+++ b/include/vaeteb.h
@@ -25,22 +25,41 @@
 int vt_get_h16_format(void);
 
 
+typedef struct {
+    float* out;
+    const int* kind;
+    const float* mean;
+    const float* stdv;
+    int first, count;
+    int C;
+    int reserved;
+} vt_fe_segment;
+typedef struct {
+    int n_seg;
+    int s0, S_len;
+    float log_eps;
+    vt_fe_segment seg[2];
+} vt_fe_epilogue;
+
 int vt_fe_spectrum(const float* x, int64_t rows, int N, int n_pad, int pad_left, int pad_mode, const void* tw,
                    void* xhat, void* stream);
+int vt_fe_spectrum_raw(const float* x, int64_t rows, int N, int n_pad, int pad_left, int pad_mode, const void* tw,
+                       void* xhat, float* raw_out, int raw_every, int raw_off, int raw_len, float mean, float stdv,
+                       void* stream);
 int vt_fe_spectrum_rolled(const float* x, int64_t B, int64_t x_row_stride, int N, int n_pad, int pad_left,
                           int pad_mode, const int* shifts, int K, const void* tw, void* xhat, void* stream);
 
 int vt_fe_lowpass(const float* x, int64_t rows, int64_t x_row_stride, int N, int n_pad, int pad_left,
                   const float* h0, int radius, int step, int start, int S, float* out, int64_t out_row_stride,
-                  void* stream);
+                  void* stream, const void* epilogue);
 
 int vt_fe_wavelet(const void* xhat, int64_t B, int C, int n_pad, const float* psi, int n_items, const int* items,
                   const void* tw, int N, int pad_left, void* analytic, int n_slots, const float* h0, int radius,
-                  int step, int start, int S, float* s1, int s1_channels, void* stream);
+                  int step, int start, int S, float* s1, int s1_channels, void* stream, const void* epilogue);
 
 int vt_fe_pairs(const void* analytic, int64_t B, int n_slots, int N, int n_pad, int pad_left, int n_pairs,
                 const int* slot_i, const int* slot_j, const float* power, const void* tw, const float* phi0, int dec,
-                int start, int S, int pad_mode, float* out, void* stream);
+                int start, int S, int pad_mode, float* out, void* stream, const void* epilogue);
 int vt_fe_pairs_split(const void* analytic_i, int n_slots_i, const void* analytic_j, int n_slots_j, int64_t B, int K,
                       int N, int n_pad, int pad_left, int n_pairs, const int* slot_i, const int* slot_j,
                       const float* power, const void* tw, const float* phi0, int dec, int start, int S,
diff --git a/vae-teb_amd/csrc/fe_norm.h b/vae-teb_amd/csrc/fe_norm.h
--- /dev/null
+++ b/vae-teb_amd/csrc/fe_norm.h
@@ -0,0 +1,45 @@
+#pragma once
+#include "common.h"
+
+namespace vt {
+
+__device__ __forceinline__ float fe_norm_val(float v, int kind, float mean, float stdv, float log_eps) {
+#pragma clang fp contract(off)
+    if (kind == 1) v = logf(fmaxf(v, 0.f) + log_eps);
+    else if (kind == 2) v = asinhf(v);
+    return (v - mean) / (stdv + 1e-8f);
+}
+
+struct FeEpiItem {
+    float* o;
+    int C, kind, s0, S_len;
+    float mean, stdv, log_eps;
+    __device__ __forceinline__ void store(int s, float v) const {
+        const int m = s - s0;
+        if (o != nullptr && m >= 0 && m < S_len) o[(int64_t)m * C] = fe_norm_val(v, kind, mean, stdv, log_eps);
+    }
+};
+
+__device__ __forceinline__ FeEpiItem fe_epi_item(const vt_fe_epilogue& e, int64_t b, int item) {
+    const bool second = e.n_seg > 1 && item >= e.seg[1].first;
+    const int first = second ? e.seg[1].first : e.seg[0].first;
+    const int count = second ? e.seg[1].count : e.seg[0].count;
+    float* out = second ? e.seg[1].out : e.seg[0].out;
+    const int* kind = second ? e.seg[1].kind : e.seg[0].kind;
+    const float* mean = second ? e.seg[1].mean : e.seg[0].mean;
+    const float* stdv = second ? e.seg[1].stdv : e.seg[0].stdv;
+    const int c = item - first;
+    const bool in = c >= 0 && c < count;
+    FeEpiItem it;
+    it.C = second ? e.seg[1].C : e.seg[0].C;
+    it.s0 = e.s0;
+    it.S_len = e.S_len;
+    it.log_eps = e.log_eps;
+    it.o = in ? out + (b * e.S_len) * (int64_t)it.C + c : nullptr;
+    it.kind = in ? kind[c] : 0;
+    it.mean = in ? mean[c] : 0.f;
+    it.stdv = in ? stdv[c] : 1.f;
+    return it;
+}
+
+}
diff --git a/vae-teb_amd/csrc/frontend.hip b/vae-teb_amd/csrc/frontend.hip
--- a/vae-teb_amd/csrc/frontend.hip
+++ b/vae-teb_amd/csrc/frontend.hip
@@ -7,6 +7,7 @@
 #include "common.h"
 #include "cfft.h"
 #include "fft.h"
+#include "fe_norm.h"
 
 namespace vt {
 
@@ -15,7 +16,9 @@
 __global__ __launch_bounds__(FE_THREADS) void k_fe_spectrum(const float* __restrict__ x, int N, int n_pad,
                                                             int pad_left, int pad_mode,
                                                             const float2* __restrict__ tw,
-                                                            float2* __restrict__ xhat) {
+                                                            float2* __restrict__ xhat, float* __restrict__ raw_out,
+                                                            int raw_every, int raw_off, int raw_len, float mean,
+                                                            float stdv) {
     extern __shared__ __attribute__((aligned(16))) float2 sm[];
     float2* X = sm;
     float2* Y = sm + n_pad;
@@ -24,6 +27,11 @@
     for (int n = threadIdx.x; n < n_pad; n += blockDim.x) {
         const int s = pad_src(n - pad_left, N, pad_mode);
         X[n] = make_float2(s < 0 ? 0.f : xr[s], 0.f);
+    }
+    if (raw_out != nullptr && row % raw_every == 0) {
+        float* ro = raw_out + (row / raw_every) * raw_len;
+        for (int i = threadIdx.x; i < raw_len; i += blockDim.x)
+            ro[i] = fe_norm_val(xr[raw_off + i], 0, mean, stdv, 0.f);
     }
     __syncthreads();
     float2* R = fft_lds<false>(X, Y, n_pad, tw, 1);
@@ -58,7 +66,8 @@
 __global__ __launch_bounds__(256) void k_fe_lowpass_lds(const float* __restrict__ x, int64_t x_row_stride, int N,
                                                         int n_pad, int pad_left, const float* __restrict__ h0,
                                                         int radius, int step, int start, int S,
-                                                        float* __restrict__ out, int64_t out_row_stride) {
+                                                        float* __restrict__ out, int64_t out_row_stride,
+                                                        const vt_fe_epilogue epi) {
     extern __shared__ float xp[];
     const int64_t row = blockIdx.y;
     const float* xr = x + row * x_row_stride;
@@ -91,12 +100,13 @@
             acc += xp[n] * h0[d < 0 ? -d : d];
         }
     }
-    out[row * out_row_stride + m] = acc;
+    if (epi.n_seg) fe_epi_item(epi, row, 0).store(m, acc);
+    else out[row * out_row_stride + m] = acc;
 }
 
 __global__ void k_fe_lowpass(const float* __restrict__ x, int64_t x_row_stride, int N, int n_pad, int pad_left,
                              const float* __restrict__ h0, int radius, int step, int start, int S,
-                             float* __restrict__ out, int64_t out_row_stride) {
+                             float* __restrict__ out, int64_t out_row_stride, const vt_fe_epilogue epi) {
     const int64_t row = blockIdx.y;
     const int m = blockIdx.x * blockDim.x + threadIdx.x;
     if (m >= S) return;
@@ -109,14 +119,15 @@
         if (n < 0) n += n_pad;
         acc += xr[reflect_idx(n - pad_left, N)] * h0[d < 0 ? -d : d];
     }
-    out[row * out_row_stride + m] = acc;
+    if (epi.n_seg) fe_epi_item(epi, row, 0).store(m, acc);
+    else out[row * out_row_stride + m] = acc;
 }
 
 __global__ __launch_bounds__(FE_THREADS) void k_fe_wavelet(
     const float2* __restrict__ xhat, int C, int n_pad, const float* __restrict__ psi, int n_items,
     const int* __restrict__ items, const float2* __restrict__ tw, int N, int pad_left, float2* __restrict__ analytic,
     int n_slots, const float* __restrict__ h0, int radius, int step, int start, int S, float* __restrict__ s1,
-    int s1_channels) {
+    int s1_channels, const vt_fe_epilogue epi) {
     extern __shared__ __attribute__((aligned(16))) float2 sm[];
     float2* X = sm;
     float2* Y = sm + n_pad;
@@ -142,6 +153,8 @@
             U[n] = sqrtf(v.x * v.x + v.y * v.y);
         }
         __syncthreads();
+        FeEpiItem ei = {};
+        if (epi.n_seg) ei = fe_epi_item(epi, b, s1ch);
         for (int m = threadIdx.x; m < S; m += blockDim.x) {
             const int c = step * (m + start);
             const int lo = (c - radius + (1 << k1) - 1) >> k1;
@@ -154,7 +167,8 @@
                 if (nn < 0) nn += M;
                 acc += U[nn] * h0[d];
             }
-            s1[(b * s1_channels + s1ch) * S + m] = acc;
+            if (epi.n_seg) ei.store(m, acc);
+            else s1[(b * s1_channels + s1ch) * S + m] = acc;
         }
     }
 }
@@ -189,7 +203,8 @@
 __device__ __forceinline__ void fe_pairs_item(const float2* ai, const float2* aj, float* __restrict__ o, const float pw,
                                               int N, int n_pad, int pad_left, const float2* __restrict__ tw,
                                               const float* __restrict__ phi0, int dec, int start, int S,
-                                              int pad_mode) {
+                                              int pad_mode, const vt_fe_epilogue& epi, const int64_t b,
+                                              const int pair) {
     extern __shared__ __attribute__((aligned(16))) float2 sm[];
     float2* X = sm;
     float2* Y = sm + n_pad;
@@ -221,6 +236,11 @@
     __syncthreads();
     float2* Rs = fft_lds<true>(Z, R, nb, tw, dec);
     const float inv = 1.0f / (float)nb;
+    if (epi.n_seg) {
+        const FeEpiItem ei = fe_epi_item(epi, b, pair);
+        for (int m = threadIdx.x; m < S; m += blockDim.x) ei.store(m, Rs[start + m].x * inv);
+        return;
+    }
     for (int m = threadIdx.x; m < S; m += blockDim.x) o[m] = Rs[start + m].x * inv;
 }
 
@@ -229,14 +249,14 @@
     const float2* __restrict__ analytic, int n_slots, int N, int n_pad, int pad_left, int n_pairs,
     const int* __restrict__ slot_i, const int* __restrict__ slot_j, const float* __restrict__ power,
     const float2* __restrict__ tw, const float* __restrict__ phi0, int dec, int start, int S, int pad_mode,
-    float* __restrict__ out) {
+    float* __restrict__ out, const vt_fe_epilogue epi) {
     const int pair = blockIdx.x;
     const int64_t b = blockIdx.y;
     const float2* ai = analytic + (b * n_slots + slot_i[pair]) * (int64_t)N;
     const float2* aj = analytic + (b * n_slots + slot_j[pair]) * (int64_t)N;
     const float pw = power[pair];
     float* o = out + (b * n_pairs + pair) * (int64_t)S;
-    fe_pairs_item<POLAR>(ai, aj, o, pw, N, n_pad, pad_left, tw, phi0, dec, start, S, pad_mode);
+    fe_pairs_item<POLAR>(ai, aj, o, pw, N, n_pad, pad_left, tw, phi0, dec, start, S, pad_mode, epi, b, pair);
 }
 
 template <bool POLAR>
@@ -251,7 +271,8 @@
     const float2* aj = analytic_j + (r * n_slots_j + slot_j[pair]) * (int64_t)N;
     const float pw = power[pair];
     float* o = out + (r * n_pairs + pair) * (int64_t)S;
-    fe_pairs_item<POLAR>(ai, aj, o, pw, N, n_pad, pad_left, tw, phi0, dec, start, S, pad_mode);
+    fe_pairs_item<POLAR>(ai, aj, o, pw, N, n_pad, pad_left, tw, phi0, dec, start, S, pad_mode, vt_fe_epilogue{}, r,
+                         pair);
 }
 
 static constexpr int PR_N = 8192, PR_NB = 512, PR_IMG = 16 * 16 * 33;
@@ -295,6 +316,12 @@
     return (total & 7) == 0 ? (L & 7) * (total >> 3) + (L >> 3) : L;
 }
 
+__device__ __forceinline__ void pr_epilogue_store(const float* V, int S, const FeEpiItem& ei, const bool epi) {
+    if (!epi) return;
+    __syncthreads();
+    for (int m = threadIdx.x; m < S; m += blockDim.x) ei.store(m, V[m]);
+}
+
 #define PR_STAMP(i)                                                              \
     do {                                                                         \
         if constexpr (P) {                                                       \
@@ -307,7 +334,8 @@
                                                 const float pw, int N_, int pad_left_,
                                                 const float2* __restrict__ tab, const float* __restrict__ phi0,
                                                 int start, int S, int pad_mode_, const int64_t b, int n_pairs,
-                                                const int pair, unsigned long long* __restrict__ stamps) {
+                                                const int pair, unsigned long long* __restrict__ stamps,
+                                                const FeEpiItem& ei, const bool epi) {
     static_assert(PR_T == 512, "one padded column per thread");
     const int N = G ? 4096 : N_, pad_left = G ? 2048 : pad_left_, pad_mode = G ? 0 : pad_mode_;
     extern __shared__ __attribute__((aligned(16))) float2 sm[];
@@ -403,6 +431,7 @@
     c2 w5[7], wb5[7];
     if (t < 64) fft512_twiddles(tab, w5, wb5);
     __syncthreads();
+    float* V = reinterpret_cast<float*>(img);
     if (t < 64) {
         c2 r[8];
         wave_fft512(Z, w5, wb5, r);
@@ -413,10 +442,14 @@
 #pragma unroll
         for (int j = 0; j < 8; ++j) {
             const int m = k0 + 64 * j - start;
-            if (m >= 0 && m < S) o[m] = r[j].x * inv;
+            if (m >= 0 && m < S) {
+                if (epi) V[m] = r[j].x * inv;
+                else o[m] = r[j].x * inv;
+            }
         }
         PR_STAMP(6);
     }
+    pr_epilogue_store(V, S, ei, epi);
 }
 #undef PR_STAMP
 
@@ -425,7 +458,7 @@
     const float2* __restrict__ analytic, int n_slots, int N_, int pad_left_, int n_pairs, int B,
     const int* __restrict__ slot_i, const int* __restrict__ slot_j, const float* __restrict__ power,
     const float2* __restrict__ tab, const float* __restrict__ phi0, int start, int S, int pad_mode_,
-    float* __restrict__ out, unsigned long long* __restrict__ stamps) {
+    float* __restrict__ out, unsigned long long* __restrict__ stamps, const vt_fe_epilogue epi) {
     const int N = G ? 4096 : N_;
     const int item = xcd_item(blockIdx.x, n_pairs * B);
     const int pair = item % n_pairs;
@@ -433,8 +466,10 @@
     const float2* ai = analytic + (b * n_slots + slot_i[pair]) * (int64_t)N;
     const float2* aj = analytic + (b * n_slots + slot_j[pair]) * (int64_t)N;
     const float pw = power[pair];
+    FeEpiItem ei = {};
+    if (epi.n_seg) ei = fe_epi_item(epi, b, pair);
     fe_pairs8k_item<G, D, P, POLAR>(ai, aj, out, pw, N_, pad_left_, tab, phi0, start, S, pad_mode_, b, n_pairs, pair,
-                                    stamps);
+                                    stamps, ei, epi.n_seg != 0);
 }
 
 template <bool G, bool POLAR>
@@ -451,7 +486,7 @@
     const float2* aj = analytic_j + (r * n_slots_j + slot_j[pair]) * (int64_t)N;
     const float pw = power[pair];
     fe_pairs8k_item<G, false, false, POLAR>(ai, aj, out, pw, N_, pad_left_, tab, phi0, start, S, pad_mode_, r,
-                                            n_pairs, pair, nullptr);
+                                            n_pairs, pair, nullptr, FeEpiItem{}, false);
 }
 
 static constexpr int PRP_T7 = PR_T - 64;
@@ -692,7 +727,8 @@
 template <bool POLAR, int OCC, int P3>
 __device__ __forceinline__ void fe_pairs8k_h_item(const float2* ai, const float2* aj, float* __restrict__ o,
                                                   const float pw, const float2* __restrict__ tab,
-                                                  const float* __restrict__ phi0, int start, int S) {
+                                                  const float* __restrict__ phi0, int start, int S,
+                                                  const FeEpiItem& ei, const bool epi) {
     extern __shared__ __attribute__((aligned(16))) float2 sm[];
     float2* img = sm;
     float2* Z = sm + PRH_BUF;
@@ -736,6 +772,7 @@
     c2 w5[7], wb5[7];
     if (t < 64) fft512_twiddles(tab, w5, wb5);
     __syncthreads();
+    float* V = reinterpret_cast<float*>(img);
     if (t < 64) {
         c2 r[8];
         wave_fft512(Z, w5, wb5, r);
@@ -744,16 +781,20 @@
 #pragma unroll
         for (int j = 0; j < 8; ++j) {
             const int m = k0 + 64 * j - start;
-            if (m >= 0 && m < S) o[m] = r[j].x * inv;
-        }
-    }
+            if (m >= 0 && m < S) {
+                if (epi) V[m] = r[j].x * inv;
+                else o[m] = r[j].x * inv;
+            }
+        }
+    }
+    pr_epilogue_store(V, S, ei, epi);
 }
 
 template <bool POLAR, int OCC, int P3 = 1>
 __global__ __launch_bounds__(PR_T) __attribute__((amdgpu_waves_per_eu(OCC, OCC))) void k_fe_pairs8k_h(
     const float2* __restrict__ analytic, int n_slots, int n_pairs, int B, const int* __restrict__ slot_i,
     const int* __restrict__ slot_j, const float* __restrict__ power, const float2* __restrict__ tab,
-    const float* __restrict__ phi0, int start, int S, float* __restrict__ out) {
+    const float* __restrict__ phi0, int start, int S, float* __restrict__ out, const vt_fe_epilogue epi) {
     constexpr int N = 4096;
     const int item = xcd_item(blockIdx.x, n_pairs * B);
     const int pair = item % n_pairs;
@@ -761,7 +802,10 @@
     const float2* ai = analytic + (b * n_slots + slot_i[pair]) * (int64_t)N;
     const float2* aj = analytic + (b * n_slots + slot_j[pair]) * (int64_t)N;
     const float pw = power[pair];
-    fe_pairs8k_h_item<POLAR, OCC, P3>(ai, aj, out + (b * n_pairs + pair) * (int64_t)S, pw, tab, phi0, start, S);
+    FeEpiItem ei = {};
+    if (epi.n_seg) ei = fe_epi_item(epi, b, pair);
+    fe_pairs8k_h_item<POLAR, OCC, P3>(ai, aj, out + (b * n_pairs + pair) * (int64_t)S, pw, tab, phi0, start, S, ei,
+                                      epi.n_seg != 0);
 }
 
 template <bool POLAR, int OCC, int P3 = 1>
@@ -777,17 +821,18 @@
     const float2* ai = analytic_i + ((r / K) * n_slots_i + slot_i[pair]) * (int64_t)N;
     const float2* aj = analytic_j + (r * n_slots_j + slot_j[pair]) * (int64_t)N;
     const float pw = power[pair];
-    fe_pairs8k_h_item<POLAR, OCC, P3>(ai, aj, out + (r * n_pairs + pair) * (int64_t)S, pw, tab, phi0, start, S);
+    fe_pairs8k_h_item<POLAR, OCC, P3>(ai, aj, out + (r * n_pairs + pair) * (int64_t)S, pw, tab, phi0, start, S,
+                                      FeEpiItem{}, false);
 }
 
 __device__ __forceinline__ int nat_pos(int k) { return k + (k >> 5); }
 
-template <bool POLAR, bool LP = true>
+template <bool POLAR, bool LP = true, bool EPI = false>
 __global__ __launch_bounds__(PR_T) void k_fe_wavelet8k(
     const float2* __restrict__ xhat, int C, const float* __restrict__ psi, const int* __restrict__ items, int n_items,
     int B, const float2* __restrict__ tab, int N, int pad_left, float2* __restrict__ analytic, int n_slots,
     const float* __restrict__ h0, int radius, int step, int start, int S, float* __restrict__ s1, int s1_channels,
-    int nowrap) {
+    int nowrap, const vt_fe_epilogue epi) {
     static_assert(PR_T == 512, "one column per thread");
     extern __shared__ __attribute__((aligned(16))) float2 sm[];
     float2* img = sm;
@@ -799,6 +844,14 @@
     const int s1ch = items[item * 5 + 3], k1 = items[item * 5 + 4];
     const float2* xh = xhat + (b * C + chan) * (int64_t)PR_N;
     const float* ps = psi + (int64_t)filt * PR_N;
+    FeEpiItem ei = {};
+    if constexpr (EPI) {
+        if (s1ch >= 0) ei = fe_epi_item(epi, b, s1ch);
+    }
+    auto put_s1 = [&](int m, float acc) {
+        if constexpr (EPI) ei.store(m, acc);
+        else s1[(b * s1_channels + s1ch) * S + m] = acc;
+    };
     {
         c2 v[16], w[15];
 #pragma unroll
@@ -891,14 +944,14 @@
                     const int nn = c0 + j;
                     acc = fmaf(img[nat_pos(nn << k1)].x, h0[(j < 0 ? -j : j) << k1], acc);
                 }
-                s1[(b * s1_channels + s1ch) * S + m] = acc;
+                put_s1(m, acc);
             }
         } else {
             for (int m = t; m < S; m += PR_T) {
                 const int c = step * (m + start);
                 const int lo = (c - radius + (1 << k1) - 1) >> k1;
                 const int hi = (c + radius) >> k1;
-                s1[(b * s1_channels + s1ch) * S + m] = taps(c, lo, hi);
+                put_s1(m, taps(c, lo, hi));
             }
         }
     } else if (s1ch >= 0) {
@@ -919,7 +972,7 @@
                 const float2 u = img[nat_pos(nn << k1)];
                 acc += sqrtf(u.x * u.x + u.y * u.y) * h0[d];
             }
-            s1[(b * s1_channels + s1ch) * S + m] = acc;
+            put_s1(m, acc);
         }
     }
 }
@@ -932,18 +985,15 @@
     const int idx = blockIdx.x * blockDim.x + threadIdx.x;
     if (idx >= C * S) return;
     const int c = idx % C, s = idx / C;
-    float v = in[(b * in_C + c) * in_S + s0 + s];
-    const int k = kind[c];
-    if (k == 1) v = logf(fmaxf(v, 0.f) + log_eps);
-    else if (k == 2) v = asinhf(v);
-    out[(b * S + s) * out_C + out_off + c] = (v - mean[c]) / (stdv[c] + 1e-8f);
+    const float v = in[(b * in_C + c) * in_S + s0 + s];
+    out[(b * S + s) * out_C + out_off + c] = fe_norm_val(v, kind[c], mean[c], stdv[c], log_eps);
 }
 
 __global__ void k_normalize_raw(const float* __restrict__ x, int64_t row_stride, int N, float mean, float stdv,
                                 float* __restrict__ out) {
     const int64_t r = blockIdx.y;
     const int i = blockIdx.x * blockDim.x + threadIdx.x;
-    if (i < N) out[r * N + i] = (x[r * row_stride + i] - mean) / (stdv + 1e-8f);
+    if (i < N) out[r * N + i] = fe_norm_val(x[r * row_stride + i], 0, mean, stdv, 0.f);
 }
 
 __global__ __launch_bounds__(FE_THREADS) void k_fft_rows(const float2* __restrict__ in, float2* __restrict__ out,
@@ -1095,20 +1145,44 @@
 }
 static inline size_t fft_lds_bytes(int n) { return (size_t)2 * n * sizeof(float2); }
 
+static bool fe_epilogue(const void* p, int n_items, int S_out, vt_fe_epilogue* e) {
+    *e = vt_fe_epilogue{};
+    if (p == nullptr) return true;
+    *e = *(const vt_fe_epilogue*)p;
+    if (e->n_seg < 1 || e->n_seg > 2 || e->s0 < 0 || e->S_len <= 0 || e->s0 + e->S_len > S_out) return false;
+    for (int i = 0; i < e->n_seg; ++i) {
+        const vt_fe_segment& g = e->seg[i];
+        if (g.out == nullptr || g.kind == nullptr || g.mean == nullptr || g.stdv == nullptr) return false;
+        if (g.first < 0 || g.count <= 0 || g.first + g.count > n_items || g.C < g.count) return false;
+    }
+    if (e->n_seg == 2 && e->seg[0].first + e->seg[0].count > e->seg[1].first) return false;
+    if (e->n_seg == 1) e->seg[1] = vt_fe_segment{};
+    return true;
+}
+
 }
 
 using namespace vt;
 
 extern "C" {
+
+int vt_fe_spectrum_raw(const float* x, int64_t rows, int N, int n_pad, int pad_left, int pad_mode, const void* tw,
+                       void* xhat, float* raw_out, int raw_every, int raw_off, int raw_len, float mean, float stdv,
+                       void* stream) {
+    VT_CHECK_ARG(pow2(n_pad) && n_pad <= VT_FFT_MAX_LDS && n_pad >= N, "vt_fe_spectrum: n_pad=%d", n_pad);
+    VT_CHECK_ARG(rows > 0 && N > 1 && pad_mode >= 0 && pad_mode <= 2, "vt_fe_spectrum: rows/N/pad_mode");
+    VT_CHECK_ARG(raw_out == nullptr || (raw_every >= 1 && raw_off >= 0 && raw_len > 0 && raw_off + raw_len <= N),
+                 "vt_fe_spectrum_raw: raw_every/raw_off/raw_len");
+    hipLaunchKernelGGL(k_fe_spectrum, dim3((unsigned)rows), dim3(FE_THREADS), fft_lds_bytes(n_pad), S(stream), x, N,
+                       n_pad, pad_left, pad_mode, (const float2*)tw, (float2*)xhat, raw_out, raw_every, raw_off,
+                       raw_len, mean, stdv);
+    VT_LAUNCH_CHECK("vt_fe_spectrum");
+    return VT_OK;
+}
 
 int vt_fe_spectrum(const float* x, int64_t rows, int N, int n_pad, int pad_left, int pad_mode, const void* tw,
                    void* xhat, void* stream) {
-    VT_CHECK_ARG(pow2(n_pad) && n_pad <= VT_FFT_MAX_LDS && n_pad >= N, "vt_fe_spectrum: n_pad=%d", n_pad);
-    VT_CHECK_ARG(rows > 0 && N > 1 && pad_mode >= 0 && pad_mode <= 2, "vt_fe_spectrum: rows/N/pad_mode");
-    hipLaunchKernelGGL(k_fe_spectrum, dim3((unsigned)rows), dim3(FE_THREADS), fft_lds_bytes(n_pad), S(stream), x, N,
-                       n_pad, pad_left, pad_mode, (const float2*)tw, (float2*)xhat);
-    VT_LAUNCH_CHECK("vt_fe_spectrum");
-    return VT_OK;
+    return vt_fe_spectrum_raw(x, rows, N, n_pad, pad_left, pad_mode, tw, xhat, nullptr, 1, 0, 0, 0.f, 1.f, stream);
 }
 
 int vt_fe_spectrum_rolled(const float* x, int64_t B, int64_t x_row_stride, int N, int n_pad, int pad_left,
@@ -1128,15 +1202,18 @@
 
 int vt_fe_lowpass(const float* x, int64_t rows, int64_t x_row_stride, int N, int n_pad, int pad_left,
                   const float* h0, int radius, int step, int start, int S_out, float* out, int64_t out_row_stride,
-                  void* stream) {
+                  void* stream, const void* epilogue) {
     VT_CHECK_ARG(rows > 0 && S_out > 0 && radius >= 0, "vt_fe_lowpass: shape");
+    vt_fe_epilogue epi;
+    VT_CHECK_ARG(fe_epilogue(epilogue, 1 << 30, S_out, &epi) && (epi.n_seg == 0 || epi.seg[0].first == 0),
+                 "vt_fe_lowpass: epilogue");
     dim3 grid((S_out + 255) / 256, (unsigned)rows);
     if ((size_t)n_pad * sizeof(float) <= 64 * 1024)
         hipLaunchKernelGGL(k_fe_lowpass_lds, grid, dim3(256), (size_t)n_pad * sizeof(float), S(stream), x, x_row_stride,
-                           N, n_pad, pad_left, h0, radius, step, start, S_out, out, out_row_stride);
+                           N, n_pad, pad_left, h0, radius, step, start, S_out, out, out_row_stride, epi);
     else
         hipLaunchKernelGGL(k_fe_lowpass, grid, dim3(256), 0, S(stream), x, x_row_stride, N, n_pad, pad_left, h0,
-                           radius, step, start, S_out, out, out_row_stride);
+                           radius, step, start, S_out, out, out_row_stride, epi);
     VT_LAUNCH_CHECK("vt_fe_lowpass");
     return VT_OK;
 }
@@ -1159,9 +1236,11 @@
 
 int vt_fe_wavelet(const void* xhat, int64_t B, int C, int n_pad, const float* psi, int n_items, const int* items,
                   const void* tw, int N, int pad_left, void* analytic, int n_slots, const float* h0, int radius,
-                  int step, int start, int S_out, float* s1, int s1_channels, void* stream) {
+                  int step, int start, int S_out, float* s1, int s1_channels, void* stream, const void* epilogue) {
     VT_CHECK_ARG(pow2(n_pad) && n_pad <= VT_FFT_MAX_LDS, "vt_fe_wavelet: n_pad=%d", n_pad);
     VT_CHECK_ARG(B > 0 && n_items > 0, "vt_fe_wavelet: empty");
+    vt_fe_epilogue epi;
+    VT_CHECK_ARG(fe_epilogue(epilogue, s1_channels, S_out, &epi), "vt_fe_wavelet: epilogue");
     VT_CHECK_ARG(step * start - radius >= 0, "vt_fe_wavelet: lowpass window leaves the padded support");
     if (n_pad == PR_N && pad_left + N <= PR_N) {
         const int nowrap = step * (start + S_out - 1) + radius < n_pad ? 1 : 0;
@@ -1173,14 +1252,18 @@
         const bool pol = analytic_polar(n_pad, N, pad_left);
         auto kern = pol ? (lp ? k_fe_wavelet8k<true, true> : k_fe_wavelet8k<true, false>)
                         : (lp ? k_fe_wavelet8k<false, true> : k_fe_wavelet8k<false, false>);
+        if (epi.n_seg)
+            kern = pol ? (lp ? k_fe_wavelet8k<true, true, true> : k_fe_wavelet8k<true, false, true>)
+                       : (lp ? k_fe_wavelet8k<false, true, true> : k_fe_wavelet8k<false, false, true>);
         const size_t lds = PR_IMG * sizeof(float2) + (lp ? (size_t)((radius + 4) / 4 * 4) * 4 : 0);
         hipLaunchKernelGGL(kern, dim3((unsigned)(n_items * B)), dim3(PR_T), lds,
                            S(stream), (const float2*)xhat, C, psi, items, n_items, (int)B, tab, N, pad_left,
-                           (float2*)analytic, n_slots, h0, radius, step, start, S_out, s1, s1_channels, nowrap);
+                           (float2*)analytic, n_slots, h0, radius, step, start, S_out, s1, s1_channels, nowrap, epi);
     } else {
         hipLaunchKernelGGL(k_fe_wavelet, dim3(n_items, (unsigned)B), dim3(FE_THREADS), fft_lds_bytes(n_pad),
                            S(stream), (const float2*)xhat, C, n_pad, psi, n_items, items, (const float2*)tw, N,
-                           pad_left, (float2*)analytic, n_slots, h0, radius, step, start, S_out, s1, s1_channels);
+                           pad_left, (float2*)analytic, n_slots, h0, radius, step, start, S_out, s1, s1_channels,
+                           epi);
     }
     VT_LAUNCH_CHECK("vt_fe_wavelet");
     return VT_OK;
@@ -1250,8 +1333,12 @@
 
 int vt_fe_pairs(const void* analytic, int64_t B, int n_slots, int N, int n_pad, int pad_left, int n_pairs,
                 const int* slot_i, const int* slot_j, const float* power, const void* tw, const float* phi0, int dec,
-                int start, int S_out, int pad_mode, float* out, void* stream) {
+                int start, int S_out, int pad_mode, float* out, void* stream, const void* epilogue) {
     VT_CHECK_ARG(pow2(n_pad) && n_pad <= VT_FFT_MAX_LDS, "vt_fe_pairs: n_pad=%d", n_pad);
+    vt_fe_epilogue epi;
+    VT_CHECK_ARG(fe_epilogue(epilogue, n_pairs, S_out, &epi) && (epi.n_seg == 0 || dec != 0),
+                 "vt_fe_pairs: epilogue (segments within the pairs and kept steps; needs the low-pass)");
+    const bool fused = epi.n_seg != 0;
     VT_CHECK_ARG(dec == 0 ? S_out == N : (dec >= 1 && pow2(dec) && n_pad / dec >= start + S_out),
                  "vt_fe_pairs: dec/start (decimation must be a power of two)");
     VT_CHECK_ARG(B > 0 && n_pairs > 0 && pad_mode >= 0 && pad_mode <= 2, "vt_fe_pairs: empty/pad_mode");
@@ -1263,14 +1350,14 @@
                                : k_fe_pairs8k<false, false, false, true>)
                         : (geo ? (direct ? k_fe_pairs8k<true, true, false, false> : k_fe_pairs8k<true, false, false, false>)
                                : k_fe_pairs8k<false, false, false, false>);
-        if (g_pairs_stamps != nullptr && geo && !direct)
+        if (g_pairs_stamps != nullptr && geo && !direct && !fused)
             kern = pol ? k_fe_pairs8k<true, false, true, true> : k_fe_pairs8k<true, false, true, false>;
         const float2* tab = tw8k_tables(S(stream));
         VT_CHECK_ARG(tab != nullptr, "vt_fe_pairs: twiddle tables unavailable (first call under stream capture?)");
         VT_CHECK_ARG((int64_t)n_pairs * B < (1ll << 31), "vt_fe_pairs: grid");
         const int64_t total = (int64_t)n_pairs * B;
         const int pgrid = pairs_persist_grid();
-        if (geo && !direct && g_pairs_stamps == nullptr && pgrid > 0 && total >= 2 * pgrid) {
+        if (geo && !direct && g_pairs_stamps == nullptr && pgrid > 0 && total >= 2 * pgrid && !fused) {
             hipLaunchKernelGGL(pol ? k_fe_pairs8k_p<true> : k_fe_pairs8k_p<false>, dim3((unsigned)pgrid), dim3(PR_T),
                                (PR_IMG + PR_ZP) * sizeof(float2),
                                S(stream), (const float2*)analytic, n_slots, n_pairs, (int)B, slot_i, slot_j, power, tab,
@@ -1288,19 +1375,19 @@
                                                 : k_fe_pairs8k_h<false, 6>),
                                dim3((unsigned)total), dim3(PR_T),
                                PRH_LDS, S(stream), (const float2*)analytic, n_slots, n_pairs, (int)B, slot_i, slot_j,
-                               power, tab, phi0, start, S_out, out);
+                               power, tab, phi0, start, S_out, out, epi);
             VT_LAUNCH_CHECK("vt_fe_pairs");
             return VT_OK;
         }
         hipLaunchKernelGGL(kern, dim3((unsigned)(n_pairs * B)), dim3(PR_T), (PR_IMG + PR_ZP) * sizeof(float2),
                            S(stream), (const float2*)analytic, n_slots, N, pad_left, n_pairs, (int)B, slot_i, slot_j,
-                           power, tab, phi0, start, S_out, pad_mode, out, g_pairs_stamps);
-        if (g_pairs_stamps != nullptr && geo && !direct) g_pairs_stamps += (size_t)B * n_pairs * 8;
+                           power, tab, phi0, start, S_out, pad_mode, out, fused ? nullptr : g_pairs_stamps, epi);
+        if (g_pairs_stamps != nullptr && geo && !direct && !fused) g_pairs_stamps += (size_t)B * n_pairs * 8;
     } else {
         hipLaunchKernelGGL(analytic_polar(n_pad, N, pad_left) ? k_fe_pairs<true> : k_fe_pairs<false>,
                            dim3(n_pairs, (unsigned)B), dim3(FE_THREADS), fft_lds_bytes(n_pad), S(stream),
                            (const float2*)analytic, n_slots, N, n_pad, pad_left, n_pairs, slot_i, slot_j, power,
-                           (const float2*)tw, phi0, dec, start, S_out, pad_mode, out);
+                           (const float2*)tw, phi0, dec, start, S_out, pad_mode, out, epi);
     }
     VT_LAUNCH_CHECK("vt_fe_pairs");
     return VT_OK;
diff --git a/vae-teb_amd/vaeteb/frontend.py b/vae-teb_amd/vaeteb/frontend.py
--- a/vae-teb_amd/vaeteb/frontend.py
+++ b/vae-teb_amd/vaeteb/frontend.py
@@ -1,4 +1,6 @@
+import ctypes
 import math
+import os
 
 import numpy as np
 import torch
@@ -105,41 +107,83 @@
 PAD_MODES = {"reflect": 0, "constant": 1, "circular": 2}
 
 
-def launch_spectrum(p, x, rows, pad_mode, xhat):
-    _lib.call("vt_fe_spectrum", _lib.ptr(x), rows, p.N, p.n_pad, p.pad_left, pad_mode, _lib.ptr(p.t_tw),
-              _lib.ptr(xhat), _lib.stream())
-
-
-def launch_lowpass(p, x, rows, x_row_stride, out, out_row_stride):
+class _Segment(ctypes.Structure):
+    _fields_ = [("out", ctypes.c_void_p), ("kind", ctypes.c_void_p), ("mean", ctypes.c_void_p),
+                ("stdv", ctypes.c_void_p), ("first", ctypes.c_int), ("count", ctypes.c_int), ("C", ctypes.c_int),
+                ("reserved", ctypes.c_int)]
+
+
+class _Epilogue(ctypes.Structure):
+    _fields_ = [("n_seg", ctypes.c_int), ("s0", ctypes.c_int), ("S_len", ctypes.c_int), ("log_eps", ctypes.c_float),
+                ("seg", _Segment * 2)]
+
+
+def epilogue(B, s0, S_len, segments, log_eps=1e-6):
+    e = _Epilogue(n_seg=len(segments), s0=s0, S_len=S_len, log_eps=log_eps)
+    for g, (out, (k, m, sd), first, count) in zip(e.seg, segments):
+        if out.dim() != 3 or out.shape[0] != B or out.shape[1] != S_len or out.shape[2] < count:
+            raise ValueError(f"epilogue output {tuple(out.shape)} is not ({B}, {S_len}, >= {count})")
+        g.out, g.kind, g.mean, g.stdv = _lib.ptr(out), _lib.ptr(k), _lib.ptr(m), _lib.ptr(sd)
+        g.first, g.count, g.C = first, count, out.shape[2]
+    return e
+
+
+def _epi_arg(e):
+    return None if e is None else ctypes.addressof(e)
+
+
+def launch_spectrum(p, x, rows, pad_mode, xhat, raw=None):
+    if raw is None:
+        _lib.call("vt_fe_spectrum", _lib.ptr(x), rows, p.N, p.n_pad, p.pad_left, pad_mode, _lib.ptr(p.t_tw),
+                  _lib.ptr(xhat), _lib.stream())
+    else:
+        out, every, off, length, mean, std = raw
+        _lib.call("vt_fe_spectrum_raw", _lib.ptr(x), rows, p.N, p.n_pad, p.pad_left, pad_mode, _lib.ptr(p.t_tw),
+                  _lib.ptr(xhat), _lib.ptr(out), every, off, length, mean, std, _lib.stream())
+
+
+def launch_lowpass(p, x, rows, x_row_stride, out, out_row_stride, epi=None):
     _lib.call("vt_fe_lowpass", _lib.ptr(x), rows, x_row_stride, p.N, p.n_pad, p.pad_left, _lib.ptr(p.t_h0), p.radius,
-              p.step, p.start, p.S, out.data_ptr(), out_row_stride, _lib.stream())
-
-
-def launch_wavelet(p, xhat, B, C, tab, analytic, s1, s1_channels):
+              p.step, p.start, p.S, out.data_ptr() if out is not None else None, out_row_stride, _lib.stream(),
+              _epi_arg(epi))
+
+
+def launch_wavelet(p, xhat, B, C, tab, analytic, s1, s1_channels, epi=None):
     _lib.call("vt_fe_wavelet", _lib.ptr(xhat), B, C, p.n_pad, _lib.ptr(p.t_psi), tab["n_items"], _lib.ptr(tab["items"]),
               _lib.ptr(p.t_tw), p.N, p.pad_left, _lib.ptr(analytic) if analytic is not None else None,
               max(tab["n_slots"], 1), _lib.ptr(p.t_h0), p.radius, p.step, p.start, p.S,
-              _lib.ptr(s1) if s1 is not None else None, s1_channels, _lib.stream())
-
-
-def launch_pairs(p, analytic, B, tab, out, lowpass=True, pad_mode=0):
+              _lib.ptr(s1) if s1 is not None else None, s1_channels, _lib.stream(), _epi_arg(epi))
+
+
+def launch_pairs(p, analytic, B, tab, out, lowpass=True, pad_mode=0, epi=None):
     if lowpass:
         _lib.call("vt_fe_pairs", _lib.ptr(analytic), B, tab["n_slots"], p.N, p.n_pad, p.pad_left, tab["n_pairs"],
                   _lib.ptr(tab["slot_i"]), _lib.ptr(tab["slot_j"]), _lib.ptr(tab["power"]), _lib.ptr(p.t_tw),
-                  _lib.ptr(p.t_phi_crop), p.dec, p.pair_start, p.pair_len, pad_mode, _lib.ptr(out), _lib.stream())
+                  _lib.ptr(p.t_phi_crop), p.dec, p.pair_start, p.pair_len, pad_mode, _lib.ptr(out), _lib.stream(),
+                  _epi_arg(epi))
     else:
         _lib.call("vt_fe_pairs", _lib.ptr(analytic), B, tab["n_slots"], p.N, p.n_pad, p.pad_left, tab["n_pairs"],
                   _lib.ptr(tab["slot_i"]), _lib.ptr(tab["slot_j"]), _lib.ptr(tab["power"]), _lib.ptr(p.t_tw),
-                  _lib.ptr(p.t_phi_crop), 0, 0, p.N, pad_mode, _lib.ptr(out), _lib.stream())
+                  _lib.ptr(p.t_phi_crop), 0, 0, p.N, pad_mode, _lib.ptr(out), _lib.stream(), None)
 
 
 class FrontEnd:
 
-    def __init__(self, plan: FrontEndPlan, stats=None, trim=0):
+    FUSABLE = ("raw", "st", "pairs")
+    FUSED_DEFAULT = ("raw", "pairs")
+
+    def __init__(self, plan: FrontEndPlan, stats=None, trim=0, fused=None):
         self.plan = p = plan
         if trim < 0 or 2 * trim >= p.S:
             raise ValueError(f"trim {trim} out of range for {p.S} steps")
         self.trim = trim
+        if fused is None:
+            env = os.environ.get("VAETEB_FE_FUSED")
+            fused = self.FUSED_DEFAULT if env is None else [n for n in env.split(",") if n]
+        if set(fused) - set(self.FUSABLE):
+            raise ValueError(f"fused: {sorted(set(fused) - set(self.FUSABLE))} not in {self.FUSABLE}")
+        self.fused = frozenset(fused)
+        self._epis = {}
         self.S_out = p.S - 2 * trim
         self.N_out = p.N - 2 * trim * p.step
         self.phase_pairs = np.nonzero(p.phase_mask)[0]
@@ -164,6 +208,7 @@
             s[f] = (_i32(k, dev), _f32(m, dev), _f32(np.sqrt(v), dev))
         s["fhr"] = (float(np.asarray(stats["fhr_mean"])), float(np.sqrt(np.asarray(stats["fhr_variance"]))))
         self.stats = s
+        self._epis = {}
 
     def fit_stats(self, batches, side=None):
         from .stats import StatsAccumulator
@@ -183,66 +228,96 @@
         return b
 
     def raw(self, x, side=None):
+        return self._run(x, side, None)
+
+    def _epi(self, key, B, segments):
+        key = (key, B) + tuple(o.data_ptr() for o, *_ in segments)
+        e = self._epis.get(key)
+        if e is None:
+            if len(self._epis) > 64:
+                self._epis.clear()
+            e = self._epis[key] = epilogue(B, self.trim, self.S_out, segments)
+        return e
+
+    def _run(self, x, side, y):
         p, t = self.plan, self.tab
         if x.dim() != 3 or x.shape[1] != 2 or x.shape[2] != p.N:
             raise ValueError(f"expected (B, 2, {p.N}) windows, got {tuple(x.shape)}")
         x = x.contiguous()
         B = x.shape[0]
+        f = self.fused if y is not None else frozenset()
         xhat = self._buf("xhat", (B, 2, p.n_pad, 2))
-        launch_spectrum(p, x, B * 2, 0, xhat)
-        s_raw = self._buf("s_raw", (B, self.C_st, p.S))
-        launch_lowpass(p, x, B, 2 * p.N, s_raw, self.C_st * p.S)
+        raw_out = (y["fhr"], 2, self.trim * p.step, self.N_out, *self.stats["fhr"]) if "raw" in f else None
+        launch_spectrum(p, x, B * 2, 0, xhat, raw=raw_out)
+        e_st = self._epi("st", B, [(y["fhr_st"], self.stats["fhr_st"], 0, self.C_st)]) if "st" in f else None
+        s_raw = None if e_st is not None else self._buf("s_raw", (B, self.C_st, p.S))
+        launch_lowpass(p, x, B, 2 * p.N, s_raw, self.C_st * p.S, epi=e_st)
         an = self._buf("analytic", (B, t["n_slots"], p.N, 2))
-        launch_wavelet(p, xhat, B, 2, t, an, s_raw, self.C_st)
+        launch_wavelet(p, xhat, B, 2, t, an, s_raw, self.C_st, epi=e_st)
+        fp = "pairs" in f
+        seg_ph = lambda: (y["fhr_ph"], self.stats["fhr_ph"], 0, self.C_ph)
         if side is None or not self.C_ph or not self.C_x:
-            pr = self._buf("pairs", (B, t["n_pairs"], p.pair_len))
-            launch_pairs(p, an, B, t, pr, lowpass=True, pad_mode=0)
+            if fp:
+                segs = ([seg_ph()] if self.C_ph else []) + \
+                       ([(y["fhr_up_ph"], self.stats["fhr_up_ph"], self.C_ph, self.C_x)] if self.C_x else [])
+                pr = None
+                launch_pairs(p, an, B, t, None, lowpass=True, pad_mode=0, epi=self._epi("pairs", B, segs))
+            else:
+                pr = self._buf("pairs", (B, t["n_pairs"], p.pair_len))
+                launch_pairs(p, an, B, t, pr, lowpass=True, pad_mode=0)
             return {"fhr_st": s_raw, "pairs": pr}
         main = torch.cuda.current_stream()
         side.wait_stream(main)
-        pr = self._buf("pairs_ph", (B, self.C_ph, p.pair_len))
-        launch_pairs(p, an, B, _sub_table(t, 0, self.C_ph), pr, lowpass=True, pad_mode=0)
+        pr = None if fp else self._buf("pairs_ph", (B, self.C_ph, p.pair_len))
+        launch_pairs(p, an, B, _sub_table(t, 0, self.C_ph), pr, lowpass=True, pad_mode=0,
+                     epi=self._epi("phase", B, [seg_ph()]) if fp else None)
         with torch.cuda.stream(side):
-            px = self._buf("pairs_x", (B, self.C_x, p.pair_len))
-            launch_pairs(p, an, B, _sub_table(t, self.C_ph, self.C_x), px, lowpass=True, pad_mode=0)
+            px = None if fp else self._buf("pairs_x", (B, self.C_x, p.pair_len))
+            launch_pairs(p, an, B, _sub_table(t, self.C_ph, self.C_x), px, lowpass=True, pad_mode=0,
+                         epi=self._epi("cross", B, [(y["fhr_up_ph"], self.stats["fhr_up_ph"], 0, self.C_x)]) if fp
+                         else None)
         return {"fhr_st": s_raw, "pairs": pr, "cross": px}
 
     def __call__(self, x, out=None, side=None):
         if self.stats is None:
             raise RuntimeError("FrontEnd needs normalisation statistics (set_stats)")
         p = self.plan
-        r = self.raw(x, side)
         B, S, S0, Sl = x.shape[0], p.S, self.trim, self.S_out
-        st = _lib.stream()
         out = {} if out is None else out
         get = lambda k, shape: out[k] if k in out else torch.empty(shape, device=p.device)
         y_st = get("fhr_st", (B, Sl, self.C_st))
         y_ph = get("fhr_ph", (B, Sl, self.C_ph))
         x_ph = get("fhr_up_ph", (B, Sl, self.C_x))
         y_raw = get("fhr", (B, self.N_out))
-        k, m, s = self.stats["fhr_st"]
-        _lib.call("vt_fe_normalize_window", _lib.ptr(r["fhr_st"]), B, self.C_st, self.C_st, S, S0, Sl, _lib.ptr(k),
-                  _lib.ptr(m), _lib.ptr(s), 1e-6, _lib.ptr(y_st), self.C_st, 0, st)
+        y = {"fhr_st": y_st, "fhr_ph": y_ph, "fhr_up_ph": x_ph, "fhr": y_raw}
+        r = self._run(x, side, y)
+        st = _lib.stream()
+        if r["fhr_st"] is not None:
+            k, m, s = self.stats["fhr_st"]
+            _lib.call("vt_fe_normalize_window", _lib.ptr(r["fhr_st"]), B, self.C_st, self.C_st, S, S0, Sl,
+                      _lib.ptr(k), _lib.ptr(m), _lib.ptr(s), 1e-6, _lib.ptr(y_st), self.C_st, 0, st)
         pairs = r["pairs"]
-        if self.C_ph:
+        if self.C_ph and pairs is not None:
             k, m, s = self.stats["fhr_ph"]
             _lib.call("vt_fe_normalize_window", pairs.data_ptr(), B, self.C_ph, pairs.shape[1], S, S0, Sl,
                       _lib.ptr(k), _lib.ptr(m), _lib.ptr(s), 1e-6, _lib.ptr(y_ph), self.C_ph, 0, st)
         if self.C_x:
             k, m, s = self.stats["fhr_up_ph"]
             if "cross" in r:
-                with torch.cuda.stream(side):
-                    _lib.call("vt_fe_normalize_window", r["cross"].data_ptr(), B, self.C_x, self.C_x, S, S0, Sl,
-                              _lib.ptr(k), _lib.ptr(m), _lib.ptr(s), 1e-6, _lib.ptr(x_ph), self.C_x, 0,
-                              _lib.stream())
+                if r["cross"] is not None:
+                    with torch.cuda.stream(side):
+                        _lib.call("vt_fe_normalize_window", r["cross"].data_ptr(), B, self.C_x, self.C_x, S, S0, Sl,
+                                  _lib.ptr(k), _lib.ptr(m), _lib.ptr(s), 1e-6, _lib.ptr(x_ph), self.C_x, 0,
+                                  _lib.stream())
                 x_ph.record_stream(side)
-            else:
+            elif pairs is not None:
                 _lib.call("vt_fe_normalize_window", pairs[:, self.C_ph:].data_ptr(), B, self.C_x, pairs.shape[1], S,
                           S0, Sl, _lib.ptr(k), _lib.ptr(m), _lib.ptr(s), 1e-6, _lib.ptr(x_ph), self.C_x, 0, st)
-        fm, fs = self.stats["fhr"]
-        _lib.call("vt_normalize_raw", _lib.ptr(x) + 4 * S0 * p.step, B, 2 * p.N, self.N_out, fm, fs, _lib.ptr(y_raw),
-                  st)
-        return {"fhr_st": y_st, "fhr_ph": y_ph, "fhr_up_ph": x_ph, "fhr": y_raw}
+        if "raw" not in self.fused:
+            fm, fs = self.stats["fhr"]
+            _lib.call("vt_normalize_raw", _lib.ptr(x) + 4 * S0 * p.step, B, 2 * p.N, self.N_out, fm, fs,
+                      _lib.ptr(y_raw), st)
+        return y
 
 
 def _sub_table(t, first, count):
```

New measurement: 33860, median of 6. Within noise of the previous version (+0.6%).
